# Sharath-girish/Shacira

Hardware: AMD Instinct MI355X
Metric: hash-grid samples/sec fwd+bwd (16 lvl, F=2) (higher is better)
Workload: dtype f32

## Files before the change

### shacira_amd/csrc/api.hip

```cpp
#include <atomic>
#include <cmath>
#include <cstdint>
#include <cstring>

#include "internal.h"

namespace shacira {

struct OptionSlot {
    const char *name;
    int Options::*field;
    int lo, hi;
    std::atomic<int> value;
};
static OptionSlot g_slots[] = {
    {"fwd_variant", &Options::fwd_variant, -1, 9, {-1}},
    {"bwd_variant", &Options::bwd_variant, -1, 1, {-1}},
    {"mlp_variant", &Options::mlp_variant, -1, 1, {-1}},
    {"bwd_compact", &Options::bwd_compact, 0, 1, {1}},
    {"bwd_selective_zero", &Options::bwd_selective_zero, 0, 1, {1}},
    {"bwd_persistent", &Options::bwd_persistent, 0, 1, {1}},
    {"bwd_fork", &Options::bwd_fork, 0, 1, {1}},
    {"bwd_run_pad", &Options::bwd_run_pad, 0, 1, {1}},
    {"bwd_item12", &Options::bwd_item12, -1, 1, {-1}},
    {"bin_acc_kib", &Options::bin_acc_kib, 0, 128, {0}},
    {"bin_batch_mib", &Options::bin_batch_mib, 1, 1 << 20, {1536}},
    {"tiled", &Options::tiled, -1, 1, {-1}},
    {"tiled_lc_fwd", &Options::tiled_lc_fwd, -1, SHACIRA_MAX_LODS, {-1}},
    {"bwd_brick", &Options::bwd_brick, -1, 1, {-1}},
    {"bwd_brick_lo", &Options::bwd_brick_lo, -1, SHACIRA_MAX_LODS, {-1}},
    {"bwd_brick_hi", &Options::bwd_brick_hi, -1, SHACIRA_MAX_LODS, {-1}},
    {"bwd_brick_fork", &Options::bwd_brick_fork, 0, 2, {2}},
    {"bwd_brick_span", &Options::bwd_brick_span, 0, 64, {0}},
    {"fwd_direct", &Options::fwd_direct, -1, 1, {-1}},
    {"bwd_ext_fork", &Options::bwd_ext_fork, 0, 1, {1}},
    {"coord_variant", &Options::coord_variant, -1, 8, {-1}},
    {"triplane_layout", &Options::triplane_layout, -1, 1, {-1}},
};
static thread_local Options tl_options;
const Options &opt() { return tl_options; }
void options_snapshot() {
    for (OptionSlot &sl : g_slots) tl_options.*(sl.field) = sl.value.load(std::memory_order_relaxed);
}
void options_resolve_item12(int value) { tl_options.bwd_item12 = value; }
static bool option_value_ok(const OptionSlot &sl, int v) {
    if (v < sl.lo || v > sl.hi) return false;
    if (!std::strcmp(sl.name, "fwd_variant")) return v == -1 || v == 0 || v == 3 || v == 6 || v == 8 || v == 9;
    if (!std::strcmp(sl.name, "coord_variant")) return v == -1 || v == 0 || v == 3 || v == 8;
    if (!std::strcmp(sl.name, "bin_acc_kib")) return v == 0 || v == 64 || v == 128;
    return true;
}

static int build_level_table(int dim, int num_lods, int feature_dim, int bw, const int32_t *res_host,
                             int64_t table_rows, LevelTable &lt) {
    if (dim != 2 && dim != 3) return SHACIRA_EINVAL;
    if (num_lods < 1 || num_lods > SHACIRA_MAX_LODS) return SHACIRA_EINVAL;
    if (feature_dim < 1) return SHACIRA_EINVAL;
    if (feature_dim % 2 == 1) return SHACIRA_EODD;
    if (bw < 1 || bw > 30) return SHACIRA_EINVAL;
    if (!res_host || table_rows < 0) return SHACIRA_EINVAL;
    std::memset(&lt, 0, sizeof(lt));
    const int32_t cs = (int32_t)std::pow(2.0, (double)bw);
    for (int l = 0; l < num_lods; ++l) {
        const int32_t r = res_host[l];
        if (r < 1) return SHACIRA_EINVAL;
        lt.res[l] = r;
        lt.hi[l] = (float)((double)r - 1.0 - 1e-5);
        lt.dense[l] = level_is_dense(dim, r, cs) ? 1 : 0;
    }
    lt.mask = (uint32_t)cs - 1u;
    lt.num_lods = num_lods;
    lt.feature_dim = feature_dim;
    lt.table_rows = table_rows;
    lt.level_begin = 0;
    lt.level_end = num_lods;
    lt.stage_flags = 0;
    return 0;
}

}

using namespace shacira;

extern "C" {

int shacira_abi_version(void) { return SHACIRA_ABI_VERSION; }

const char *shacira_strerror(int code) {
    switch (code) {
        case 0: return "success";
        case SHACIRA_EINVAL: return "shacira: invalid argument (dim/sizes/bitwidth/null pointer)";
        case SHACIRA_EDTYPE: return "shacira: unsupported scalar type or operator shape";
        case SHACIRA_EODD: return "The codebook feature dimension needs to be a multiple of 2.";
        case SHACIRA_EWORKSPACE: return "shacira: workspace too small";
        default: break;
    }
    if (code > 0) return hipGetErrorString((hipError_t)code);
    return "shacira: unknown error";
}

int shacira_set_option(const char *name, int value) {
    if (!name) return SHACIRA_EINVAL;
    for (OptionSlot &sl : g_slots) {
        if (std::strcmp(name, sl.name)) continue;
        if (!option_value_ok(sl, value)) return SHACIRA_EINVAL;
        sl.value.store(value, std::memory_order_relaxed);
        return 0;
    }
    return SHACIRA_EINVAL;
}

int shacira_get_option(const char *name) {
    if (!name) return SHACIRA_EINVAL;
    for (OptionSlot &sl : g_slots)
        if (!std::strcmp(name, sl.name)) return sl.value.load(std::memory_order_relaxed);
    return SHACIRA_EINVAL;
}

size_t shacira_hashgrid_forward_workspace_bytes(int dim, int64_t num_coords, int num_lods, int feature_dim,
                                                int codebook_bitwidth, const int32_t *resolutions_host,
                                                int64_t table_rows, int dtype) {
    options_snapshot();
    LevelTable lt;
    if (build_level_table(dim, num_lods, feature_dim, codebook_bitwidth, resolutions_host, table_rows, lt)) return 0;
    return hashgrid_forward_workspace(dim, dtype, lt, num_coords);
}

int shacira_hashgrid_forward(int dim, int64_t num_coords, int num_lods, int feature_dim, int codebook_bitwidth,
                             const int32_t *resolutions_host, const int32_t *codebook_first_idx, int64_t table_rows,
                             const float *coords, const void *codebook, int dtype, void *feats, void *workspace,
                             size_t workspace_bytes, void *stream) {
    return shacira_hashgrid_forward_planned(dim, num_coords, num_lods, feature_dim, codebook_bitwidth, resolutions_host,
                                            codebook_first_idx, table_rows, coords, codebook, dtype, feats, nullptr, 0, 0,
                                            workspace, workspace_bytes, stream);
}

size_t shacira_hashgrid_plan_bytes(int dim, int64_t num_coords, int num_lods, int feature_dim, int codebook_bitwidth,
                                   const int32_t *resolutions_host, int64_t table_rows, int dtype) {
    options_snapshot();
    LevelTable lt;
    if (build_level_table(dim, num_lods, feature_dim, codebook_bitwidth, resolutions_host, table_rows, lt)) return 0;
    if (dtype == SHACIRA_F64 || table_rows == 0 || !tiled_supported(dim, dtype, lt, num_coords)) return 0;
    return sample_plan_bytes(dim, num_coords);
}

int shacira_hashgrid_forward_planned(int dim, int64_t num_coords, int num_lods, int feature_dim, int codebook_bitwidth,
                                     const int32_t *resolutions_host, const int32_t *codebook_first_idx, int64_t table_rows,
                                     const float *coords, const void *codebook, int dtype, void *feats, void *plan,
                                     size_t plan_bytes, int plan_flags, void *workspace, size_t workspace_bytes,
                                     void *stream) {
    options_snapshot();
    LevelTable lt;
    int rc = build_level_table(dim, num_lods, feature_dim, codebook_bitwidth, resolutions_host, table_rows, lt);
    if (rc) return rc;
    if (dtype != SHACIRA_F32 && dtype != SHACIRA_F16 && dtype != SHACIRA_F64) return SHACIRA_EDTYPE;
    if (num_coords < 0) return SHACIRA_EINVAL;
    if (num_coords == 0) return 0;
    if (!codebook_first_idx || !coords || !codebook || !feats) return SHACIRA_EINVAL;
    const size_t need = hashgrid_forward_workspace(dim, dtype, lt, num_coords);
    if (need > 0 && (!workspace || workspace_bytes < need)) return SHACIRA_EWORKSPACE;
    const bool sorts = dtype != SHACIRA_F64 && table_rows > 0 && tiled_supported(dim, dtype, lt, num_coords);
    if (plan != nullptr && sorts && plan_bytes < sample_plan_bytes(dim, num_coords)) return SHACIRA_EWORKSPACE;
    if ((plan_flags & ~SHACIRA_PLAN_READY) != 0 || ((plan_flags & SHACIRA_PLAN_READY) != 0 && plan == nullptr)) return SHACIRA_EINVAL;
    return (int)hashgrid_forward_dispatch(dim, dtype, lt, codebook_first_idx, coords, codebook, feats, workspace,
                                          num_coords, (hipStream_t)stream, sorts ? plan : nullptr,
                                          (plan_flags & SHACIRA_PLAN_READY) != 0);
}

int shacira_hashgrid_debug_corners(int dim, int64_t num_coords, int num_lods, int codebook_bitwidth,
                                   const int32_t *resolutions_host, const float *coords, int32_t *corner_rows,
                                   float *corner_weights, void *stream) {
    LevelTable lt;
    int rc = build_level_table(dim, num_lods, 2, codebook_bitwidth, resolutions_host, 0, lt);
    if (rc) return rc;
    if (num_coords < 0 || num_coords * (int64_t)num_lods >= ((int64_t)1 << 31) * 256) return SHACIRA_EINVAL;
    if (num_coords > 0 && (!coords || (!corner_rows && !corner_weights))) return SHACIRA_EINVAL;
    return (int)hashgrid_debug_corners(dim, lt, coords, num_coords, corner_rows, corner_weights, (hipStream_t)stream);
}

size_t shacira_hashgrid_backward_workspace_bytes(int dim, int64_t num_coords, int num_lods, int feature_dim,
                                                 int codebook_bitwidth, const int32_t *resolutions_host,
                                                 int64_t table_rows, int dtype) {
    options_snapshot();
    LevelTable lt;
    if (build_level_table(dim, num_lods, feature_dim, codebook_bitwidth, resolutions_host, table_rows, lt)) return 0;
    return hashgrid_backward_workspace(dim, dtype, lt, num_coords);
}

int shacira_hashgrid_backward(int dim, int64_t num_coords, int num_lods, int feature_dim, int codebook_bitwidth,
                              const int32_t *resolutions_host, const int32_t *codebook_first_idx, int64_t table_rows,
                              const float *coords, const void *grad_output, int dtype, void *grad_codebook,
                              void *workspace, size_t workspace_bytes, void *stream) {
    return shacira_hashgrid_backward_levels(dim, num_coords, num_lods, feature_dim, codebook_bitwidth, resolutions_host,
                                            codebook_first_idx, table_rows, coords, grad_output, dtype, grad_codebook,
                                            0, num_lods, 0, workspace, workspace_bytes, stream);
}

static int backward_call(int dim, int64_t num_coords, int num_lods, int feature_dim, int codebook_bitwidth,
                         const int32_t *resolutions_host, const int32_t *codebook_first_idx, int64_t table_rows,
                         const float *coords, const void *grad_output, int dtype, void *grad_codebook, int level_begin,
                         int level_end, int flags, const void *plan, size_t plan_bytes, void *workspace,
                         size_t workspace_bytes, void *stream);

size_t shacira_hashgrid_backward_planned_workspace_bytes(int dim, int64_t num_coords, int num_lods, int feature_dim,
                                                         int codebook_bitwidth, const int32_t *resolutions_host,
                                                         int64_t table_rows, int dtype) {
    options_snapshot();
    LevelTable lt;
    if (build_level_table(dim, num_lods, feature_dim, codebook_bitwidth, resolutions_host, table_rows, lt)) return 0;
    LevelTable full = lt;
    const bool sorts = dtype != SHACIRA_F64 && table_rows > 0 && tiled_supported(dim, dtype, full, num_coords);
    if (!sorts) return hashgrid_backward_workspace(dim, dtype, lt, num_coords);
    return hashgrid_backward_workspace_planned(dim, dtype, lt, num_coords, true);
}

int shacira_hashgrid_backward_planned(int dim, int64_t num_coords, int num_lods, int feature_dim, int codebook_bitwidth,
                                      const int32_t *resolutions_host, const int32_t *codebook_first_idx, int64_t table_rows,
                                      const float *coords, const void *grad_output, int dtype, void *grad_codebook,
                                      const void *plan, size_t plan_bytes, void *workspace, size_t workspace_bytes,
                                      void *stream) {
    return backward_call(dim, num_coords, num_lods, feature_dim, codebook_bitwidth, resolutions_host, codebook_first_idx,
                         table_rows, coords, grad_output, dtype, grad_codebook, 0, num_lods, 0, plan, plan_bytes, workspace,
                         workspace_bytes, stream);
}

int shacira_hashgrid_backward_levels(int dim, int64_t num_coords, int num_lods, int feature_dim, int codebook_bitwidth,
                                     const int32_t *resolutions_host, const int32_t *codebook_first_idx,
                                     int64_t table_rows, const float *coords, const void *grad_output, int dtype,
                                     void *grad_codebook, int level_begin, int level_end, int flags, void *workspace,
                                     size_t workspace_bytes, void *stream) {
    return backward_call(dim, num_coords, num_lods, feature_dim, codebook_bitwidth, resolutions_host, codebook_first_idx,
                         table_rows, coords, grad_output, dtype, grad_codebook, level_begin, level_end, flags, nullptr, 0,
                         workspace, workspace_bytes, stream);
}

size_t shacira_hashgrid_coords_backward_workspace_bytes(int dim, int64_t num_coords, int num_lods, int feature_dim,
                                                        int codebook_bitwidth, const int32_t *resolutions_host,
                                                        int64_t table_rows, int dtype) {
    (void)dim; (void)num_coords; (void)num_lods; (void)feature_dim; (void)codebook_bitwidth; (void)resolutions_host;
    (void)table_rows; (void)dtype;
    return 0;
}

int shacira_hashgrid_coords_backward(int dim, int64_t num_coords, int num_lods, int feature_dim, int codebook_bitwidth,
                                     const int32_t *resolutions_host, const int32_t *codebook_first_idx, int64_t table_rows,
                                     const float *coords, const void *codebook, const void *grad_output, int dtype,
                                     float *grad_coords, const void *plan, size_t plan_bytes, void *workspace,
                                     size_t workspace_bytes, void *stream) {
    options_snapshot();
    LevelTable lt;
    int rc = build_level_table(dim, num_lods, feature_dim, codebook_bitwidth, resolutions_host, table_rows, lt);
    if (rc) return rc;
    if (dtype != SHACIRA_F32 && dtype != SHACIRA_F16 && dtype != SHACIRA_F64) return SHACIRA_EDTYPE;
    if (num_coords < 0) return SHACIRA_EINVAL;
    if (num_coords == 0) return 0;
    if (!codebook_first_idx || !coords || !codebook || !grad_output || !grad_coords) return SHACIRA_EINVAL;
    const size_t need = shacira_hashgrid_coords_backward_workspace_bytes(dim, num_coords, num_lods, feature_dim,
                                                                         codebook_bitwidth, resolutions_host, table_rows,
                                                                         dtype);
    if (need > 0 && (!workspace || workspace_bytes < need)) return SHACIRA_EWORKSPACE;
    if (plan != nullptr) {
        const bool sorts = dtype != SHACIRA_F64 && table_rows > 0 && tiled_supported(dim, dtype, lt, num_coords);
        if (!sorts) plan = nullptr;
        else if (plan_bytes < sample_plan_bytes(dim, num_coords)) return SHACIRA_EWORKSPACE;
    }
    return (int)hashgrid_coord_grad_dispatch(dim, dtype, lt, codebook_first_idx, coords, codebook, grad_output, grad_coords,
                                             num_coords, (hipStream_t)stream, plan);
}

static int triplane_args(int64_t num_coords, int num_lods, const int32_t *lods_host, int feature_dim, TriplaneArgs &a) {
    if (num_coords < 0 || num_coords > (int64_t)INT32_MAX) return SHACIRA_EINVAL;
    if (num_lods < 1 || num_lods > SHACIRA_TRIPLANE_MAX_LODS || !lods_host) return SHACIRA_EINVAL;
    if (feature_dim < 1 || feature_dim > SHACIRA_TRIPLANE_MAX_FDIM) return SHACIRA_EINVAL;
    std::memset(&a, 0, sizeof(a));
    a.num_lods = num_lods;
    a.fdim = feature_dim;
    for (int l = 0; l < num_lods; ++l) {
        if (lods_host[l] < 0 || lods_host[l] > SHACIRA_TRIPLANE_MAX_LOD) return SHACIRA_EINVAL;
        a.side[l] = (1 << lods_host[l]) + 1;
    }
    return 0;
}

static int triplane_pointers(int num_lods, const float *const *host, TriplaneArgs &a, bool grad) {
    if (!host) return SHACIRA_EINVAL;
    for (int q = 0; q < 3 * num_lods; ++q) {
        if (!host[q]) return SHACIRA_EINVAL;
        if (grad) a.grad[q] = const_cast<float *>(host[q]);
        else a.plane[q] = host[q];
    }
    return 0;
}

size_t shacira_triplane_forward_workspace_bytes(int64_t num_coords, int num_lods, const int32_t *lods_host,
                                                int feature_dim, int multiscale_sum) {
    options_snapshot();
    TriplaneArgs a;
    if (triplane_args(num_coords, num_lods, lods_host, feature_dim, a)) return 0;
    return triplane_forward_workspace(a, num_coords);
}

int shacira_triplane_forward(int64_t num_coords, int num_lods, const int32_t *lods_host, int feature_dim,
                             const float *coords, const float *const *planes_host, int multiscale_sum, float *feats,
                             void *workspace, size_t workspace_bytes, void *stream) {
    options_snapshot();
    TriplaneArgs a;
    if (int rc = triplane_args(num_coords, num_lods, lods_host, feature_dim, a)) return rc;
    if (multiscale_sum != 0 && multiscale_sum != 1) return SHACIRA_EINVAL;
    if (num_coords == 0) return 0;
    if (!coords || !feats) return SHACIRA_EINVAL;
    if (int rc = triplane_pointers(num_lods, planes_host, a, false)) return rc;
    const size_t need = triplane_forward_workspace(a, num_coords);
    if (need > 0 && (!workspace || workspace_bytes < need)) return SHACIRA_EWORKSPACE;
    return (int)triplane_forward_dispatch(a, coords, multiscale_sum, feats, workspace, num_coords, (hipStream_t)stream);
}

size_t shacira_triplane_backward_workspace_bytes(int64_t num_coords, int num_lods, const int32_t *lods_host,
                                                 int feature_dim, int multiscale_sum, int flags) {
    TriplaneArgs a;
    if (triplane_args(num_coords, num_lods, lods_host, feature_dim, a)) return 0;
    if ((flags & SHACIRA_TRIPLANE_GRAD_PLANES) == 0) return 0;
    return triplane_backward_workspace(a, multiscale_sum, num_coords);
}

int shacira_triplane_backward(int64_t num_coords, int num_lods, const int32_t *lods_host, int feature_dim,
                              const float *coords, const float *const *planes_host, const float *grad_output,
                              int multiscale_sum, int flags, float *const *grad_planes_host, float *grad_coords,
                              void *workspace, size_t workspace_bytes, void *stream) {
    TriplaneArgs a;
    if (int rc = triplane_args(num_coords, num_lods, lods_host, feature_dim, a)) return rc;
    if (multiscale_sum != 0 && multiscale_sum != 1) return SHACIRA_EINVAL;
    if (flags <= 0 || (flags & ~(SHACIRA_TRIPLANE_GRAD_PLANES | SHACIRA_TRIPLANE_GRAD_COORDS)) != 0) return SHACIRA_EINVAL;
    const bool planes = (flags & SHACIRA_TRIPLANE_GRAD_PLANES) != 0;
    const bool want_coords = (flags & SHACIRA_TRIPLANE_GRAD_COORDS) != 0;
    if (planes)
        if (int rc = triplane_pointers(num_lods, const_cast<const float *const *>(grad_planes_host), a, true)) return rc;
// ... 539 lines not shown
```

### shacira_amd/csrc/bwd_bin_front.h

```cpp
#pragma once

#include "bwd_bin_types.h"

namespace shacira {

template <typename T, int F, bool GMAX>
__global__ __launch_bounds__(256) void transpose_grad_kernel(const T *__restrict__ go, float *__restrict__ gT,
                                                             int64_t N, int64_t NP, int L, int lb, int le,
                                                             uint32_t *__restrict__ gmax) {
    __shared__ uint32_t s_max[SHACIRA_MAX_LODS];
    if (GMAX && threadIdx.x < SHACIRA_MAX_LODS) s_max[threadIdx.x] = 0;
    struct alignas(sizeof(T) * F) PieceIn { T v[F]; };
    struct alignas(sizeof(float) * F) PieceOut { float v[F]; };
    extern __shared__ __align__(16) unsigned char s_raw_g[];
    PieceOut *s_tile = reinterpret_cast<PieceOut *>(s_raw_g);
    const int pitch = L + 1;
    const int64_t s0 = (int64_t)blockIdx.x * 256;
    const int ns = (int)((N - s0 < 256) ? (N - s0) : 256);
    const PieceIn *in = reinterpret_cast<const PieceIn *>(go) + s0 * L;
    const int total = ns * L;
    for (int e = threadIdx.x; e < total; e += 256) {
        const int sm = e / L, l = e - sm * L;
        const PieceIn p = in[e];
        PieceOut q;
#pragma unroll
        for (int j = 0; j < F; ++j) q.v[j] = Scalar<T>::load(&p.v[j]);
        s_tile[sm * pitch + l] = q;
    }
    __syncthreads();
    PieceOut *out = reinterpret_cast<PieceOut *>(gT);
    for (int l = lb; l < le; ++l) {
        uint32_t m = 0;
        if ((int)threadIdx.x < ns) {
            const PieceOut q = s_tile[threadIdx.x * pitch + l];
            if constexpr (GMAX) {
#pragma unroll
                for (int j = 0; j < F; ++j) {
                    const uint32_t b = __float_as_uint(fabsf(q.v[j]));
                    m = b > m ? b : m;
                }
            }
            float *dst = reinterpret_cast<float *>(out + (int64_t)l * NP + s0 + threadIdx.x);
            if constexpr (F == 2) {
                typedef float f32x2 __attribute__((ext_vector_type(2)));
                f32x2 v = {q.v[0], q.v[1]};
                __builtin_nontemporal_store(v, reinterpret_cast<f32x2 *>(dst));
            } else {
#pragma unroll
                for (int j = 0; j < F; ++j) __builtin_nontemporal_store(q.v[j], dst + j);
            }
        }
        if constexpr (GMAX) {
#pragma unroll
            for (int off = 32; off > 0; off >>= 1) {
                const uint32_t o = __shfl_xor(m, off, 64);
                m = o > m ? o : m;
            }
            if ((threadIdx.x & 63) == 0 && m) atomicMax(&s_max[l], m);
        }
    }
    if constexpr (GMAX) {
        __syncthreads();
        if ((int)threadIdx.x >= lb && (int)threadIdx.x < le && s_max[threadIdx.x])
            atomicMax(&gmax[threadIdx.x], s_max[threadIdx.x]);
    }
}

constexpr int kFrontThreads = 512;
template <int DIM, typename T, int F, bool GMAX, bool COUNT, bool SORTED = false>
__global__ __launch_bounds__(kFrontThreads) void front16_kernel(LevelTable lt, BinPlan plan, const T *__restrict__ go,
                                                                float *__restrict__ gT, const float *__restrict__ coords,
                                                                uint32_t *__restrict__ totals, uint32_t *__restrict__ cnt,
                                                                int64_t N, int64_t NP, int lb, int le, int ts_log2,
                                                                int rounds, uint32_t *__restrict__ gmax, uint32_t cps,
                                                                const float4 *__restrict__ sorted4 = nullptr) {
    constexpr int K = 16 / (int)(sizeof(T) * F);
    constexpr int HE = SHACIRA_MAX_LODS * kMaxLevelBuckets / kFrontThreads;
    constexpr int M = 16 / (4 * F);
    constexpr int M_LOG2 = (M == 2) ? 1 : 0;
    constexpr int UL = 8;
    static_assert(K >= 1 && (M == 1 || M == 2), "16-byte transpose: F = 2 or 4");
    typedef uint32_t u32x4 __attribute__((ext_vector_type(4)));
    typedef float f32x4 __attribute__((ext_vector_type(4)));
    struct alignas(sizeof(float) * F) PieceOut { float v[F]; };
    __shared__ uint32_t s_max[SHACIRA_MAX_LODS];
    __shared__ uint32_t s_idx[SORTED ? kFrontThreads : 1];
    extern __shared__ __align__(16) unsigned char s_raw_g[];
    const int L = lt.num_lods;
    const int TS = 1 << ts_log2;
    const int pitch = TS + 2;
    PieceOut *s_tile = reinterpret_cast<PieceOut *>(s_raw_g);
    uint32_t *s_hist = reinterpret_cast<uint32_t *>(s_raw_g + (size_t)L * pitch * sizeof(PieceOut));
    if (GMAX && threadIdx.x < SHACIRA_MAX_LODS) s_max[threadIdx.x] = 0;
    if constexpr (COUNT)
        for (uint32_t k = threadIdx.x; k < plan.nbl * (uint32_t)kMaxLevelBuckets; k += kFrontThreads) s_hist[k] = 0;
    __syncthreads();
    const int VPR = L / K;
    const int nvec_log2 = ts_log2 - M_LOG2;
    const int q512 = kFrontThreads / VPR, r512 = kFrontThreads % VPR;
    const int sm_first = (int)threadIdx.x / VPR, v_first = (int)threadIdx.x % VPR;
    const int cslots = kFrontThreads >> ts_log2, csm = (int)threadIdx.x & (TS - 1);
    const int cslot = __builtin_amdgcn_readfirstlane((int)threadIdx.x >> ts_log2);
    const int64_t tile0 = (int64_t)blockIdx.x * rounds;
    const int64_t tiles = (N + TS - 1) >> ts_log2;
    uint32_t hsum[HE];
    uint32_t hacc[HE];
    static_assert(!COUNT || kFrontThreads % kMaxLevelBuckets == 0, "a wave maps to one level slot");
    const uint32_t hli0 = (uint32_t)__builtin_amdgcn_readfirstlane((int)(threadIdx.x / kMaxLevelBuckets));
    const uint32_t hb = threadIdx.x % kMaxLevelBuckets;
    auto hcol_of = [&](int j) -> int {
        const uint32_t li = hli0 + (uint32_t)j * (kFrontThreads / kMaxLevelBuckets);
        const uint32_t lc = li < (uint32_t)SHACIRA_MAX_LODS ? li : 0u;
        const uint32_t nbq = li < plan.nbl ? plan.bnb[lc] : 0u, bsq = plan.bstart[lc];
        return (hb < nbq) ? (int)(bsq + hb) : -1;
    };
    if constexpr (COUNT) {
#pragma unroll
        for (int j = 0; j < HE; ++j) {
            hsum[j] = 0;
            hacc[j] = 0;
        }
    }
    float cc[DIM];
    uint32_t cidx = 0;
    auto load_coords = [&](int r) {
        int64_t t = tile0 + r;
        if (t >= tiles) t = tiles - 1;
        const int64_t s0r = t << ts_log2;
        const int nsr = (int)((N - s0r < TS) ? (N - s0r) : TS);
        const int64_t ci = s0r + (csm < nsr ? csm : nsr - 1);
        if constexpr (SORTED) {
            const float4 rc = sorted4[ci];
            cc[0] = rc.x;
            cc[1] = rc.y;
            if constexpr (DIM == 3) cc[2] = rc.z;
            cidx = __float_as_uint(rc.w);
        } else {
#pragma unroll
            for (int a = 0; a < DIM; ++a) cc[a] = coords[ci * DIM + a];
        }
    };
    if constexpr (COUNT || SORTED) {
        if (tile0 < tiles) load_coords(0);
    }
    for (int r = 0; r < rounds && tile0 + r < tiles; ++r) {
        const int64_t s0 = (tile0 + r) << ts_log2;
        const int ns = (int)((N - s0 < TS) ? (N - s0) : TS);
        const int total = ns * VPR;
        const u32x4 *in = reinterpret_cast<const u32x4 *>(go) + (SORTED ? 0 : s0 * VPR);
        if constexpr (SORTED) {
            if (cslot == 0) s_idx[csm] = cidx;
            lds_barrier();
        }
        auto src_of = [&](int e, int smq, int vq) -> const u32x4 * {
            if constexpr (SORTED) return in + (uint32_t)(s_idx[smq] * (uint32_t)VPR + (uint32_t)vq);
            else return in + e;
        };
        u32x4 raw[UL];
        {
            int smq = sm_first, vq = v_first;
#pragma unroll
            for (int u = 0; u < UL; ++u) {
                const int e = (int)threadIdx.x + u * kFrontThreads;
                const bool in_tile = e < total;
                raw[u] = __builtin_nontemporal_load(in_tile ? src_of(e, smq, vq) : src_of(total - 1, ns - 1, VPR - 1));
                smq += q512;
                vq += r512;
                if (vq >= VPR) { vq -= VPR; ++smq; }
            }
        }
        if constexpr (COUNT || SORTED) {
            double t[DIM];
#pragma unroll
            for (int a = 0; a < DIM; ++a) t[a] = axis_unit(cc[a]);
            load_coords(r + 1);
            if (COUNT && csm < ns) {
#pragma unroll 2
                for (uint32_t li = (uint32_t)cslot; li < plan.nbl; li += (uint32_t)cslots)
                    count_level<DIM>(t, plan.cl[li], lt.mask, s_hist + li * kMaxLevelBuckets);
            }
        }
        auto park1 = [&](const u32x4 &rv, int sm, int v) {
            T tv[K * F];
            __builtin_memcpy(tv, &rv, 16);
#pragma unroll
            for (int k = 0; k < K; ++k) {
                PieceOut q;
#pragma unroll
                for (int j = 0; j < F; ++j) q.v[j] = Scalar<T>::load(&tv[k * F + j]);
                s_tile[(v * K + k) * pitch + sm] = q;
            }
        };
        int sm = sm_first, v = v_first;
#pragma unroll
        for (int u = 0; u < UL; ++u) {
            if ((int)threadIdx.x + u * kFrontThreads < total) park1(raw[u], sm, v);
            sm += q512;
            v += r512;
            if (v >= VPR) { v -= VPR; ++sm; }
        }
        for (int e = (int)threadIdx.x + kFrontThreads * UL; e < total; e += kFrontThreads) {
            park1(__builtin_nontemporal_load(src_of(e, sm, v)), sm, v);
            sm += q512;
            v += r512;
            if (v >= VPR) { v -= VPR; ++sm; }
        }
        lds_barrier();
        if constexpr (COUNT) {
            uint32_t *row = cnt + (size_t)(tile0 + r) * plan.total_buckets;
            const bool close = plan.pad > 1u && ((uint32_t)((tile0 + r + 1) % (int64_t)cps) == 0u || tile0 + r + 1 == tiles);
#pragma unroll
            for (int j = 0; j < HE; ++j) {
                const int hc = hcol_of(j);
                if (hc >= 0) {
                    const uint32_t h = s_hist[threadIdx.x + j * kFrontThreads];
                    s_hist[threadIdx.x + j * kFrontThreads] = 0;
                    row[hc] = h;
                    hacc[j] += h;
                    hsum[j] += h;
                    if (close) {
                        hsum[j] += (0u - hacc[j]) & (plan.pad - 1u);
                        hacc[j] = 0;
                    }
                }
            }
        }
        const int work = (le - lb) << nvec_log2;
        for (int idx = threadIdx.x; idx < work; idx += kFrontThreads) {
            const int l = lb + (idx >> nvec_log2), smo = (idx & ((1 << nvec_log2) - 1)) << M_LOG2;
            uint32_t m = 0;
            if (smo < ns) {
                const f32x4 val = *reinterpret_cast<const f32x4 *>(&s_tile[l * pitch + smo]);
                float *dst = gT + ((int64_t)l * NP + s0 + smo) * F;
                if (smo + M <= ns) {
                    if constexpr (sizeof(T) == 4) *reinterpret_cast<f32x4 *>(dst) = val;
                    else __builtin_nontemporal_store(val, reinterpret_cast<f32x4 *>(dst));
                    if constexpr (GMAX) {
#pragma unroll
                        for (int j = 0; j < 4; ++j) {
                            const uint32_t b = __float_as_uint(fabsf(val[j]));
                            m = b > m ? b : m;
                        }
                    }
                } else {
#pragma unroll
                    for (int j = 0; j < F; ++j) {
                        dst[j] = val[j];
                        if constexpr (GMAX) {
                            const uint32_t b = __float_as_uint(fabsf(val[j]));
                            m = b > m ? b : m;
                        }
                    }
                }
            }
            if constexpr (GMAX) {
#pragma unroll
                for (int off = 32; off > 0; off >>= 1) {
                    const uint32_t o = __shfl_xor(m, off, 64);
                    m = o > m ? o : m;
                }
                if ((threadIdx.x & 63) == 0 && m) atomicMax(&s_max[l], m);
            }
        }
        lds_barrier();
    }
    __syncthreads();
    if constexpr (COUNT) {
        uint32_t *mine = totals + (size_t)(blockIdx.x % kTotalShards) * kMaxBuckets;
#pragma unroll
        for (int j = 0; j < HE; ++j) {
            const int hc = hcol_of(j);
            if (hc >= 0 && hsum[j]) atomicAdd(&mine[hc], hsum[j]);
        }
    }
    if constexpr (GMAX) {
        if ((int)threadIdx.x >= lb && (int)threadIdx.x < le && s_max[threadIdx.x])
            atomicMax(&gmax[threadIdx.x], s_max[threadIdx.x]);
    }
}

__global__ __launch_bounds__(1024) void bin_scan_buckets_kernel(const uint32_t *__restrict__ totals,
                                                                uint64_t *__restrict__ base,
                                                                uint32_t *__restrict__ unit_first,
                                                                UnitDesc *__restrict__ unit_desc, uint32_t nb,
                                                                BinPlan plan,
                                                                uint32_t *__restrict__ work_counter,
                                                                unsigned long long *__restrict__ cursor,
                                                                const uint32_t *__restrict__ gmax) {
    __shared__ uint64_t s_items[kMaxBuckets + 2];
    __shared__ uint32_t s_units[kMaxBuckets + 2];
    __shared__ uint64_t s_wave_items[16];
    __shared__ uint32_t s_wave_units[16];
    const uint32_t t = threadIdx.x, lane = t & 63, wave = t >> 6;
    if (t == 0) work_counter[0] = 0;
    uint64_t c[2];
    uint32_t u[2], lv_of[2], ck[2];
#pragma unroll
    for (int k = 0; k < 2; ++k) {
        const uint32_t b = 2 * t + k;
        c[k] = 0u;
        if (b < nb)
            for (int sh = 0; sh < kTotalShards; ++sh) c[k] += totals[(size_t)sh * kMaxBuckets + b];
        uint32_t lvl = plan.blevel[0];
#pragma unroll
        for (uint32_t q = 1; q < SHACIRA_MAX_LODS; ++q)
            if (q < plan.nbl && plan.bstart[q] <= b) lvl = plan.blevel[q];
        lv_of[k] = lvl;
        ck[k] = plan.chunk;
        u[k] = (c[k] >> 32) ? (uint32_t)((c[k] + ck[k] - 1) / ck[k]) : (c[k] ? ((uint32_t)c[k] - 1u) / ck[k] + 1u : 0u);
    }
    uint64_t ci = c[0] + c[1];
    uint32_t ui = u[0] + u[1];
#pragma unroll
    for (int off = 1; off < 64; off <<= 1) {
        const uint64_t nc = __shfl_up(ci, off, 64);
        const uint32_t nu = __shfl_up(ui, off, 64);
        if (lane >= (uint32_t)off) { ci += nc; ui += nu; }
    }
    if (lane == 63) { s_wave_items[wave] = ci; s_wave_units[wave] = ui; }
    __syncthreads();
    uint64_t wc = 0;
    uint32_t wu = 0;
    for (uint32_t w = 0; w < wave; ++w) { wc += s_wave_items[w]; wu += s_wave_units[w]; }
    const uint64_t ex_items = wc + ci - (c[0] + c[1]);
    const uint32_t ex_units = wu + ui - (u[0] + u[1]);
    s_items[2 * t] = ex_items;
    s_items[2 * t + 1] = ex_items + c[0];
    s_units[2 * t] = ex_units;
    s_units[2 * t + 1] = ex_units + u[0];
    if (t == 1023) {
        s_items[kMaxBuckets] = ex_items + c[0] + c[1];
        s_units[kMaxBuckets] = ex_units + u[0] + u[1];
    }
    __syncthreads();
    for (uint32_t b = t; b <= nb; b += 1024) {
        base[b] = s_items[b];
        cursor[b] = s_items[b];
        unit_first[b] = s_units[b];
    }
#pragma unroll
    for (int k = 0; k < 2; ++k) {
        const uint32_t b = 2 * t + k;
        if (b < nb) {
            const uint32_t lvl = lv_of[k];
            const uint32_t gm = (gmax != nullptr && u[k] > 0) ? gmax[lvl] : 0u;
            for (uint32_t q = 0; q < u[k]; ++q) {
                UnitDesc d;
                d.begin = s_items[b] + (uint64_t)q * ck[k];
                const uint64_t bucket_end = s_items[b] + c[k];
                d.end = (d.begin + ck[k] < bucket_end) ? (d.begin + ck[k]) : bucket_end;
                d.bucket = b;
                d.level = lvl;
                d.single = u[k] == 1 ? 1u : 0u;
                d.gmax_bits = gm;
                unit_desc[s_units[b] + q] = d;
            }
        }
    }
}

template <int DIM>
__global__ __launch_bounds__(kBinThreads) void bin_count_levels_kernel(LevelTable lt, BinPlan plan,
                                                                       const float *__restrict__ coords,
                                                                       uint32_t *__restrict__ totals,
                                                                       uint32_t *__restrict__ cnt, int64_t sample0,
                                                                       int64_t N) {
    __shared__ uint32_t s_hist[SHACIRA_MAX_LODS][kMaxLevelBuckets];
    constexpr int kTileD = TileOf<DIM>::value;
    constexpr int SPT = kTileD / kBinThreads;
    const uint32_t tile = blockIdx.x;
    for (uint32_t e = threadIdx.x; e < plan.nbl * kMaxLevelBuckets; e += kBinThreads) (&s_hist[0][0])[e] = 0;
    double t[SPT][DIM];
    bool live[SPT];
#pragma unroll
    for (int u = 0; u < SPT; ++u) {
        const int64_t i = sample0 + (int64_t)tile * kTileD + threadIdx.x + u * kBinThreads;
        live[u] = i < N;
        load_unit_coords<DIM>(coords, i, N, t[u]);
    }
    __syncthreads();
#pragma unroll 1
    for (uint32_t bi = blockIdx.y; bi < plan.nbl; bi += gridDim.y) {
        const uint32_t lvl = plan.blevel[bi];
        const BinLevel bl = plan.lv[lvl];
        const int32_t res = lt.res[lvl];
        const float hi = lt.hi[lvl];
        const bool dense = lt.dense[lvl] != 0;
#pragma unroll
        for (int u = 0; u < SPT; ++u) {
            if (!live[u]) continue;
            if (bl.compact) {
                if constexpr (DIM == 3) {
                    atomicAdd(&s_hist[bi][axis_pos(t[u][2], res, hi) / bl.slab], 2u);
                } else {
                    atomicAdd(&s_hist[bi][compact2d_line(axis_pos(t[u][1], res, hi), (uint32_t)res) / bl.slab], 1u);
                }
                continue;
            }
            uint32_t bk[1 << (DIM - 1)];
            bool ok[1 << (DIM - 1)];
            enumerate_buckets<DIM>(t[u], res, hi, dense, lt.mask, bl, bk, ok);
#pragma unroll
            for (int q = 0; q < (1 << (DIM - 1)); ++q)
                if (ok[q]) atomicAdd(&s_hist[bi][bk[q]], 1u);
        }
    }
    __syncthreads();
    for (uint32_t bi = blockIdx.y; bi < plan.nbl; bi += gridDim.y) {
        const BinLevel bl = plan.lv[plan.blevel[bi]];
        for (uint32_t b = threadIdx.x; b < bl.nb; b += kBinThreads)
        {
            const uint32_t c = (s_hist[bi][b] + plan.pad - 1u) & ~(plan.pad - 1u);
            cnt[(size_t)tile * plan.total_buckets + bl.bucket0 + b] = s_hist[bi][b];
            if (c)
                atomicAdd(&totals[(size_t)((blockIdx.x + blockIdx.y) % kTotalShards) * kMaxBuckets + bl.bucket0 + b], c);
        }
    }
}

__global__ __launch_bounds__(256) void zero_unowned_rows_kernel(float *__restrict__ acc,
                                                                const int32_t *__restrict__ first_idx, LevelTable lt,
                                                                BinPlan plan, uint32_t *__restrict__ words,
                                                                uint32_t nwords) {
    if ((int)blockIdx.y == lt.num_lods) {
        for (uint32_t i = blockIdx.x * 256 + threadIdx.x; i < nwords; i += gridDim.x * 256) words[i] = 0u;
        return;
    }
    const int l = blockIdx.y, F = lt.feature_dim;
    const int64_t level0 = first_idx[l];
    const int64_t start = (l == 0) ? 0 : level0;
    const int64_t end = (l + 1 < lt.num_lods) ? (int64_t)first_idx[l + 1] : lt.table_rows;
    const BinLevel bl = plan.lv[l];
    const bool covered = bl.nb > 0 && bl.dgroup < 0 && lt.dense[l] == 0;
    const int64_t hole_lo = covered ? level0 : end;
    int64_t hole_hi = covered ? level0 + (int64_t)bl.used : end;
    if (hole_hi > end) hole_hi = end;
    const int64_t stride = (int64_t)gridDim.x * 256, t0 = (int64_t)blockIdx.x * 256 + threadIdx.x;
    for (int64_t e = start * F + t0; e < hole_lo * F; e += stride) acc[e] = 0.0f;
    for (int64_t e = hole_hi * F + t0; e < end * F; e += stride) acc[e] = 0.0f;
}

__global__ __launch_bounds__(256) void zero_words_kernel(uint32_t *__restrict__ p, uint32_t n) {
    for (uint32_t i = blockIdx.x * 256 + threadIdx.x; i < n; i += gridDim.x * 256) p[i] = 0u;
}

template <int F> __device__ __forceinline__ void rotate_features(const float (&a)[F], int rot, float (&r)[F]) {
    static_assert(F == 1 || F == 2 || F == 4 || F == 8, "power-of-two feature counts");
#pragma unroll
    for (int k = 0; k < F; ++k) r[k] = a[k];
#pragma unroll
    for (int bit = 1; bit < F; bit <<= 1) {
        int on = rot & bit;
        asm volatile("" : "+v"(on));
        float t[F];
#pragma unroll
        for (int k = 0; k < F; ++k) t[k] = on ? r[(k + bit) & (F - 1)] : r[k];
#pragma unroll
        for (int k = 0; k < F; ++k) r[k] = t[k];
    }
}

}
```

### shacira_amd/csrc/bwd_bin_passes.h

```cpp
#pragma once

#include "bwd_bin_types.h"

namespace shacira {

#ifdef SHACIRA_SCATTER_WAVES
#define SHACIRA_SCATTER_ATTR __attribute__((amdgpu_waves_per_eu(SHACIRA_SCATTER_WAVES)))
#else
#define SHACIRA_SCATTER_ATTR
#endif
template <int DIM, int F, int FMT, bool STREAM = true>
__global__ __launch_bounds__((ScatterThreads<DIM, F, FMT>::value)) SHACIRA_SCATTER_ATTR void bin_scatter_kernel(LevelTable lt, BinPlan plan,
                                                                  const float *__restrict__ coords,
                                                                  const float *__restrict__ gT,
                                                                  unsigned long long *__restrict__ cursor,
                                                                  const uint32_t *__restrict__ cnt, uint32_t cps,
                                                                  uint32_t cnt_rows,
                                                                  typename ItemSel<F, FMT>::type *__restrict__ items,
                                                                  int64_t sample0, int64_t N, int64_t gpitch,
                                                                  float *__restrict__ zero_acc,
                                                                  const int32_t *__restrict__ first_idx,
                                                                  const uint32_t *__restrict__ unit_first,
                                                                  int cstride = DIM) {
    typedef typename ItemSel<F, FMT>::type ItemT;
    constexpr bool H = FMT == 1;
    constexpr bool P12 = FMT == 2;
    static_assert(!P12 || (DIM == 3 && F == 2), "12-byte units: 3-D, F = 2");
    constexpr int NP = 1 << (DIM - 1);
    constexpr int kTileD = TileOf<DIM>::value;
    constexpr int kThreads = ScatterThreads<DIM, F, FMT>::value;
    constexpr int SPT = kTileD / kThreads;
    constexpr int kScatterSplit = ScatterSplit<ItemT>::value;
    constexpr int kStage = kTileD * NP / kScatterSplit;
    static_assert(kStage % 2 == 0, "two-slot items never straddle a window");
    extern __shared__ __align__(16) unsigned char s_raw[];
    ItemT *s_items = reinterpret_cast<ItemT *>(s_raw);
    uint8_t *s_bucket = reinterpret_cast<uint8_t *>(s_items + (kScatterSplit == 1 ? plan.stage_cap : (uint32_t)kStage));
    __shared__ uint32_t s_hist[kMaxLevelBuckets];
    __shared__ uint32_t s_start[kMaxLevelBuckets + 1];
    __shared__ uint64_t s_gbase[kMaxLevelBuckets];

#ifdef SCATTER_LEVEL_FAST
    const uint32_t tile = blockIdx.y, bi = blockIdx.x;
#else
    const uint32_t tile = blockIdx.x, bi = blockIdx.y;
#endif
    const uint32_t lvl = plan.blevel[bi];
    const BinLevel bl = plan.lv[lvl];
    if (threadIdx.x < kMaxLevelBuckets) s_hist[threadIdx.x] = 0;
    __syncthreads();
    const int32_t res = lt.res[lvl];
    const float hi = lt.hi[lvl];
    const bool dense = lt.dense[lvl] != 0;

    PairSlot ps[SPT][NP];
    uint32_t rank[SPT][NP];
    float fx[SPT];
    float g[SPT][F];
    float fyz[SPT][2];
    const bool compact = bl.compact != 0;
    constexpr uint32_t kCompactSlots = (DIM == 3) ? 2u : 1u;
    float craw[SPT][DIM], graw[SPT][F];
#pragma unroll
    for (int u = 0; u < SPT; ++u) {
        int64_t i = sample0 + (int64_t)tile * kTileD + threadIdx.x + u * kThreads;
        i = i < N ? i : N - 1;
#ifdef ABL_NO_LOAD
        i = (i * 2654435761ll) & 1023;
#endif
#pragma unroll
        for (int a = 0; a < DIM; ++a) craw[u][a] = coords[i * cstride + a];
        const float *gp = gT + ((int64_t)lvl * gpitch + i) * F;
        if constexpr (F == 2) {
            const float2 v = *reinterpret_cast<const float2 *>(gp);
            graw[u][0] = v.x; graw[u][1] = v.y;
        } else {
#pragma unroll
            for (int j = 0; j < F; ++j) graw[u][j] = gp[j];
        }
    }
    const bool reserver = threadIdx.x >= 64 && threadIdx.x - 64 < bl.nb;
    unsigned long long run_base = 0ull;
    if (reserver) {
        const uint32_t gb = bl.bucket0 + threadIdx.x - 64;
        const uint32_t *row = cnt + (size_t)tile * cps * plan.total_buckets + gb;
        uint32_t c = 0;
        for (uint32_t k = 0; k < cps && tile * cps + k < cnt_rows; ++k) c += row[(size_t)k * plan.total_buckets];
        c = (c + plan.pad - 1u) & ~(plan.pad - 1u);
#ifdef ABL_NO_CURSOR
        if (c) run_base = cursor[gb] + (unsigned long long)tile * c;
#else
        if (c) run_base = atomicAdd(&cursor[gb], (unsigned long long)c);
#endif
    }
#pragma unroll
    for (int u = 0; u < SPT; ++u) {
        const int k = threadIdx.x + u * kThreads;
        const int64_t i = sample0 + (int64_t)tile * kTileD + k;
        const bool live = i < N;
        double t[DIM];
#pragma unroll
        for (int a = 0; a < DIM; ++a) t[a] = axis_unit(craw[u][a]);
#pragma unroll
        for (int j = 0; j < F; ++j) g[u][j] = graw[u][j];
        if (compact) {
            if constexpr (DIM == 3) {
                int32_t pp[3];
                float ff[3], gg[3];
#pragma unroll
                for (int a = 0; a < 3; ++a) axis_transform(t[a], res, hi, pp[a], ff[a], gg[a]);
                const uint32_t r = (uint32_t)res, b = (uint32_t)pp[2] / bl.slab;
                const uint32_t local = ((uint32_t)pp[2] - b * bl.slab) * r * r + (uint32_t)pp[1] * r + (uint32_t)pp[0];
                fx[u] = ff[0];
                fyz[u][0] = ff[1];
                fyz[u][1] = ff[2];
#pragma unroll
                for (int q = 0; q < NP; ++q) {
                    ps[u][q].bucket = b;
                    ps[u][q].key = 0;
                    ps[u][q].wrest = 0.0f;
                }
                ps[u][0].key = local | (1u << 26);
            } else {
                int32_t pp[2];
                float ff[2], gg[2];
#pragma unroll
                for (int a = 0; a < 2; ++a) axis_transform(t[a], res, hi, pp[a], ff[a], gg[a]);
                const uint32_t r = (uint32_t)res, b = compact2d_line((uint32_t)pp[1], r) / bl.slab;
                const uint32_t local = ((uint32_t)pp[1] - b * bl.slab) * r + (uint32_t)pp[0];
                fx[u] = ff[0];
                fyz[u][0] = ff[1];
                fyz[u][1] = 0.0f;
                ps[u][0].bucket = b;
                ps[u][0].key = local | (1u << 26);
                ps[u][0].wrest = 0.0f;
                ps[u][1].bucket = b;
                ps[u][1].key = 0;
                ps[u][1].wrest = 0.0f;
            }
        } else {
            enumerate_pairs<DIM>(t, res, hi, dense, lt.mask, bl, plan.BR, fx[u], ps[u]);
        }
#pragma unroll
        for (int q = 0; q < NP; ++q) {
            if (!live) ps[u][q].key = 0;
            rank[u][q] = (ps[u][q].key >> 26) ? atomicAdd(&s_hist[ps[u][q].bucket], compact ? kCompactSlots : 1u) : 0u;
        }
    }
    lds_barrier();
    if (threadIdx.x < 64) {
        const uint32_t lane = threadIdx.x;
        const uint32_t pm = plan.pad - 1u;
        const uint32_t c0 = (2 * lane < bl.nb) ? ((s_hist[2 * lane] + pm) & ~pm) : 0u;
        const uint32_t c1 = (2 * lane + 1 < bl.nb) ? ((s_hist[2 * lane + 1] + pm) & ~pm) : 0u;
        uint32_t incl = c0 + c1;
#pragma unroll
        for (int off = 1; off < 64; off <<= 1) {
            const uint32_t nbr = __shfl_up(incl, off, 64);
            if (lane >= (uint32_t)off) incl += nbr;
        }
        const uint32_t excl = incl - (c0 + c1);
        if (2 * lane < bl.nb) s_start[2 * lane] = excl;
        if (2 * lane + 1 < bl.nb) s_start[2 * lane + 1] = excl + c0;
        if (lane == 63) s_start[bl.nb] = incl;
    }
    lds_barrier();
    if (kScatterSplit == 1 && plan.pad > 1u && threadIdx.x < bl.nb) {
        const uint32_t b = threadIdx.x;
        for (uint32_t pos = s_start[b] + s_hist[b]; pos < s_start[b + 1]; ++pos) {
            uint32_t *w = reinterpret_cast<uint32_t *>(&s_items[pos]);
#pragma unroll
            for (int k = 0; k < (int)(sizeof(ItemT) / 4); ++k) w[k] = 0u;
            s_bucket[pos] = (uint8_t)b;
        }
    }
    const uint32_t staged = s_start[bl.nb];
    const uint32_t n_win = (kScatterSplit == 1) ? 1u : (staged + (uint32_t)kStage - 1u) / (uint32_t)kStage;
    for (uint32_t wi = 0; wi < n_win; ++wi) {
    const uint32_t w0 = wi * (uint32_t)kStage;
#pragma unroll
    for (int u = 0; u < SPT; ++u) {
#pragma unroll
        for (int q = 0; q < NP; ++q) {
            if (ps[u][q].key >> 26) {
                const uint32_t gp = s_start[ps[u][q].bucket] + rank[u][q];
                if (kScatterSplit > 1 && gp - w0 >= (uint32_t)kStage) continue;
                const uint32_t pos = gp - w0;
                if constexpr (H && F == 4) {
                    ItemH4 it;
                    it.key = ps[u][q].key;
                    it.fx = fx[u];
                    if (compact) {
                        it.p2 = __float_as_uint(fyz[u][0]);
                        it.p3 = __float_as_uint(fyz[u][1]);
                        s_items[pos] = it;
                        ItemH4 it2;
                        it2.key = 0;
                        it2.fx = 0.0f;
                        it2.p2 = float2_to_half2_bits(g[u][0], g[u][1]);
                        it2.p3 = float2_to_half2_bits(g[u][2], g[u][3]);
                        s_items[pos + 1] = it2;
                        s_bucket[pos] = (uint8_t)ps[u][q].bucket;
                        s_bucket[pos + 1] = (uint8_t)ps[u][q].bucket;
                    } else {
                        const float w = ps[u][q].wrest;
                        it.p2 = float2_to_half2_bits(g[u][0] * w, g[u][1] * w);
                        it.p3 = float2_to_half2_bits(g[u][2] * w, g[u][3] * w);
                        s_items[pos] = it;
                        s_bucket[pos] = (uint8_t)ps[u][q].bucket;
                    }
                    continue;
                }
                if constexpr (P12) {
                    if (compact) {
                        Item12 u0, u1;
                        u0.w[0] = ps[u][q].key;
                        u0.w[1] = __float_as_uint(fx[u]);
                        u0.w[2] = __float_as_uint(fyz[u][0]);
                        u1.w[0] = __float_as_uint(fyz[u][1]);
                        u1.w[1] = __float_as_uint(g[u][0]);
                        u1.w[2] = __float_as_uint(g[u][1]);
                        s_items[pos] = u0;
                        s_items[pos + 1] = u1;
                        s_bucket[pos] = (uint8_t)ps[u][q].bucket;
                        s_bucket[pos + 1] = (uint8_t)ps[u][q].bucket;
                    } else {
                        s_items[pos] = pack_item12(ps[u][q].key, fx[u], dense, g[u][0] * ps[u][q].wrest, g[u][1] * ps[u][q].wrest);
                        s_bucket[pos] = (uint8_t)ps[u][q].bucket;
                    }
                    continue;
                }
                if constexpr (H && F == 2) {
                    if (compact) {
                        ItemHC c;
                        c.key = ps[u][q].key;
                        c.fx = (uint16_t)(fx[u] * 65536.0f);
                        c.fy = (uint16_t)(fyz[u][0] * 65536.0f);
                        c.fz = (uint16_t)(fyz[u][1] * 65536.0f);
                        c.pad = 0;
                        c.g = __floats2half2_rn(g[u][0], g[u][1]);
                        *reinterpret_cast<ItemHC *>(&s_items[pos]) = c;
                        s_bucket[pos] = (uint8_t)ps[u][q].bucket;
                        s_bucket[pos + 1] = (uint8_t)ps[u][q].bucket;
                    } else {
                        ItemH it;
                        it.key = pack_half_key(ps[u][q].key, fx[u], dense);
                        it.a = __floats2half2_rn(g[u][0] * ps[u][q].wrest, g[u][1] * ps[u][q].wrest);
                        s_items[pos] = it;
                        s_bucket[pos] = (uint8_t)ps[u][q].bucket;
                    }
                    continue;
                }
                if constexpr (!H && !P12) {
                Item<F> it;
                it.key = ps[u][q].key;
                it.fx = fx[u];
                if constexpr (DIM == 2 && !H) {
                    if (compact) {
                        uint32_t w0, w1;
                        pack_compact2d(ps[u][q].key, fx[u], fyz[u][0], w0, w1);
                        it.key = w0;
                        it.fx = __uint_as_float(w1);
#pragma unroll
                        for (int j = 0; j < F; ++j) it.a[j] = g[u][j];
                        *reinterpret_cast<Item<F> *>(&s_items[pos]) = it;
                        s_bucket[pos] = (uint8_t)ps[u][q].bucket;
                        continue;
                    }
                }
                if (compact) {
                    if constexpr (F == 2) {
                        it.a[0] = fyz[u][0];
                        it.a[1] = fyz[u][1];
                        *reinterpret_cast<Item<F> *>(&s_items[pos]) = it;
                        Item<F> it2;
                        it2.key = 0;
                        it2.fx = g[u][0];
                        it2.a[0] = g[u][1];
                        it2.a[1] = 0.0f;
                        *reinterpret_cast<Item<F> *>(&s_items[pos + 1]) = it2;
                        s_bucket[pos] = (uint8_t)ps[u][q].bucket;
                        s_bucket[pos + 1] = (uint8_t)ps[u][q].bucket;
                    } else if constexpr (F == 4) {
                        it.a[0] = fyz[u][0];
                        it.a[1] = fyz[u][1];
                        it.a[2] = g[u][0];
                        it.a[3] = g[u][1];
                        *reinterpret_cast<Item<F> *>(&s_items[pos]) = it;
                        Item<F> it2;
                        it2.key = 0;
                        it2.fx = g[u][2];
                        it2.a[0] = g[u][3];
                        it2.a[1] = 0.0f; it2.a[2] = 0.0f; it2.a[3] = 0.0f;
                        *reinterpret_cast<Item<F> *>(&s_items[pos + 1]) = it2;
                        s_bucket[pos] = (uint8_t)ps[u][q].bucket;
                        s_bucket[pos + 1] = (uint8_t)ps[u][q].bucket;
                    }
                } else {
#pragma unroll
                    for (int j = 0; j < F; ++j) it.a[j] = g[u][j] * ps[u][q].wrest;
                    *reinterpret_cast<Item<F> *>(&s_items[pos]) = it;
                    s_bucket[pos] = (uint8_t)ps[u][q].bucket;
                }
                }
            }
        }
    }
    if (wi == 0) {
        if (reserver) s_gbase[threadIdx.x - 64] = run_base;
        __syncthreads();
    } else {
        lds_barrier();
    }
    const uint32_t in_window = (kScatterSplit == 1 || staged - w0 < (uint32_t)kStage) ? (staged - w0) : (uint32_t)kStage;
#ifndef ABL_NO_STORE
    for (uint32_t pos = threadIdx.x; pos < in_window; pos += kThreads) {
        const uint32_t b = s_bucket[pos];
        store_item_nt<STREAM>(items + s_gbase[b] + (w0 + pos - s_start[b]), s_items[pos]);
    }
#endif
    if (kScatterSplit > 1 && wi + 1u < n_win) lds_barrier();
    }
    if (zero_acc != nullptr && !dense) {
        for (uint32_t b = tile; b < bl.nb; b += plan.num_tiles) {
            const uint32_t gb = bl.bucket0 + b;
            if (unit_first[gb + 1] - unit_first[gb] == 1u) continue;
            const uint32_t row0 = b * bl.rows_pb;
            const uint32_t nrows = (bl.used - row0 < bl.rows_pb) ? (bl.used - row0) : bl.rows_pb;
            float *dst = zero_acc + ((int64_t)first_idx[lvl] + row0) * F;
            for (uint32_t e = threadIdx.x; e < nrows * (uint32_t)F; e += kThreads) dst[e] = 0.0f;
        }
    }
}

#ifdef CONSUME_TRACE
__device__ unsigned long long g_consume_trace[16384 * 8];
__device__ unsigned int g_consume_trace_n;
#define CTRACE(k) do { if (threadIdx.x == 0) ctr[k] = wall_clock64(); } while (0)
#else
#define CTRACE(k) do { } while (0)
#endif
template <int F, bool FX, int FMT, class Hook>
__device__ __forceinline__ void consume_unit(const LevelTable &lt, const BinPlan &plan, const int32_t *__restrict__ first_idx,
                                             const UnitDesc d, const typename ItemSel<F, FMT>::type *__restrict__ items,
                                             float *__restrict__ grad_table, int force_atomic, int headroom, double *s_acc,
                                             Hook &&hook, __half *__restrict__ half_out = nullptr) {
    constexpr bool H = FMT == 1;
    constexpr bool P12 = FMT == 2;
    const uint32_t gb = (uint32_t)__builtin_amdgcn_readfirstlane((int)d.bucket);
    const uint32_t lvl = (uint32_t)__builtin_amdgcn_readfirstlane((int)d.level);
    const BinLevel bl = plan.lv[lvl];
    const uint32_t b = gb - bl.bucket0;
    const uint32_t r1 = (uint32_t)lt.res[lvl];
    const bool two_d = plan.pairs == 2u;
    const uint32_t row0 = bl.compact ? b * bl.slab * (two_d ? r1 : r1 * r1) : b * bl.rows_pb;
    const uint32_t nrows = (bl.used - row0 < bl.rows_pb) ? (bl.used - row0) : bl.rows_pb;

    FxScale fx{1.0, 1.0, false};
    if constexpr (FX) fx = fx_scale_of(d.gmax_bits, headroom);
    unsigned long long *s_fix = reinterpret_cast<unsigned long long *>(s_acc);
#ifdef CONSUME_TRACE
    unsigned long long ctr[8] = {0, 0, 0, 0, 0, 0, 0, 0};
    struct TraceOut {
        unsigned long long *c; UnitDesc dd;
        __device__ ~TraceOut() {
            if (threadIdx.x == 0) {
                c[5] = wall_clock64();
                const unsigned int slot = atomicAdd(&g_consume_trace_n, 1u);
                if (slot < 16384u) {
                    unsigned long long *o = g_consume_trace + (size_t)slot * 8;
                    o[0] = ((unsigned long long)dd.level << 32) | dd.bucket;
                    o[1] = dd.end - dd.begin;
                    for (int k = 0; k < 6; ++k) o[2 + k] = c[k];
                }
            }
        }
    } trace_out{ctr, d};
#endif
    CTRACE(0);
    auto zero_image = [&]() {
        for (uint32_t e = threadIdx.x; e < nrows * F; e += kConsumeThreads) s_acc[e] = 0.0;
        lds_barrier();
    };
    const uint64_t begin = d.begin, end = d.end;
    auto stream = [&](uint64_t first, uint64_t lim, uint64_t stride, auto &&load, auto &&proc) {
        uint64_t p0 = first;
        load(p0);
        CTRACE(1);
        zero_image();
        CTRACE(2);
        proc();
        CTRACE(3);
        hook();
        for (p0 += stride; p0 < lim; p0 += stride) {
            load(p0);
            proc();
        }
        CTRACE(4);
    };
    const int rot = (int)(threadIdx.x & (F - 1));
    auto add_row = [&](uint32_t row, const float (&vr)[F], float w) {
#pragma unroll
        for (int jj = 0; jj < F; ++jj) {
            const int j = (jj + rot) & (F - 1);
            const float c = vr[jj] * w;
            if (FX && fx.fixed) atomicAdd(&s_fix[row * F + j], fx_encode(c, fx.scale));
            else atomicAdd(&s_acc[row * F + j], (double)c);
        }
    };
#ifdef ABL_CONSUME_STREAM_ONLY
    uint32_t abl_sink = 0;
#endif
    auto add_pair = [&](uint32_t ra, uint32_t rb, bool va, bool vb, float fxv, const float (&a)[F]) {
#ifdef ABL_CONSUME_STREAM_ONLY
        abl_sink ^= ra ^ rb ^ (uint32_t)va ^ (uint32_t)vb ^ __float_as_uint(fxv) ^ __float_as_uint(a[0]) ^ __float_as_uint(a[F - 1]);
        if (abl_sink == 0x12345678u) s_fix[ra] = abl_sink;
        return;
#endif
        float ar[F];
        rotate_features<F>(a, rot, ar);
        if (va) add_row(ra, ar, 1.0f - fxv);
        if (vb) add_row(rb, ar, fxv);
    };
    const uint32_t r2 = r1 * r1;
    auto add_compact = [&](uint32_t base_row, float fxx, float fyy, float fzz, const float (&gg)[F]) {
        const float gxx = 1.0f - fxx, gyy = 1.0f - fyy, gzz = 1.0f - fzz;
        const float wxy[4] = {gxx * gyy, gxx * fyy, fxx * gyy, fxx * fyy};
        float gr[F];
        rotate_features<F>(gg, rot, gr);
#pragma unroll
        for (int c = 0; c < 8; ++c) {
            const uint32_t row = base_row + ((c >> 2) & 1) + ((c >> 1) & 1) * r1 + (c & 1) * r2;
            if (row >= nrows) continue;
            add_row(row, gr, wxy[c >> 1] * ((c & 1) ? fzz : gzz));
        }
    };
    typedef uint32_t u32x4 __attribute__((ext_vector_type(4)));
    typedef uint32_t u32x2 __attribute__((ext_vector_type(2)));
    if constexpr ((F == 2 || F == 4) && !H && !P12) {
        if (bl.compact && two_d) {
            const Item<F> *itf = reinterpret_cast<const Item<F> *>(items);
            constexpr int UD = 8;
            Item<F> it[UD];
            stream(begin + threadIdx.x, end, (uint64_t)kConsumeThreads * UD,
                   [&](uint64_t p0) {
#pragma unroll
                       for (int u = 0; u < UD; ++u) {
                           const uint64_t pp = p0 + (uint64_t)u * kConsumeThreads;
                           if (pp < end) it[u] = load_item_nt<F, FX>(itf + pp);
                           else it[u].key = 0;
                       }
                   },
                   [&]() {
#pragma unroll
                       for (int u = 0; u < UD; ++u) {
                           if (!(it[u].key & (1u << 13))) continue;
                           uint32_t local, qx, qy;
                           unpack_compact2d(it[u].key, __float_as_uint(it[u].fx), local, qx, qy);
                           const float q = 1.0f / 33554432.0f;
                           const float fxx = (float)qx * q, fyy = (float)qy * q;
                           const float gxx = 1.0f - fxx, gyy = 1.0f - fyy;
                           float ar[F];
                           rotate_features<F>(it[u].a, rot, ar);
                           if (local + r1 + 1u < nrows) {
                               add_row(local, ar, gxx * gyy);
                               if (qx) add_row(local + 1u, ar, fxx * gyy);
                               if (qy) {
                                   add_row(local + r1, ar, gxx * fyy);
                                   if (qx) add_row(local + r1 + 1u, ar, fxx * fyy);
                               }
                           } else {
                               if (local < nrows) add_row(local, ar, gxx * gyy);
                               if (qx && local + 1u < nrows) add_row(local + 1u, ar, fxx * gyy);
                               if (qy && local + r1 < nrows) add_row(local + r1, ar, gxx * fyy);
                           }
                       }
                   });
            lds_barrier();
            const int64_t grow0d = (int64_t)first_idx[lvl] + row0;
            for (uint32_t e = threadIdx.x; e < nrows * F; e += kConsumeThreads) {
                const int64_t grow = grow0d + e / F;
                if ((uint64_t)grow >= (uint64_t)lt.table_rows) continue;
                const float v = (FX && fx.fixed) ? fx_decode(s_fix[e], fx.inv) : (float)s_acc[e];
                if (v != 0.0f) unsafeAtomicAdd(grad_table + grow * F + (e % F), v);
            }
            return;
        }
    }
    if constexpr (F == 2 || F == 4) {
        if (bl.compact) {
            constexpr int UC = 2;
            const uint64_t first = begin + 2ull * threadIdx.x, stride = 2ull * kConsumeThreads * UC;
            if constexpr (P12) {
                Item12 ia[UC], ib[UC];
                uint64_t pcur = 0;
                stream(first, end, stride,
                       [&](uint64_t p0) {
                           pcur = p0;
#pragma unroll
                           for (int u = 0; u < UC; ++u) {
                               const uint64_t p = p0 + 2ull * u * kConsumeThreads;
                               const uint64_t pc = (p + 1 < end) ? p : begin;
                               ia[u] = load_item12_nt(items + pc);
                               ib[u] = load_item12_nt(items + pc + 1);
                           }
                       },
                       [&]() {
#pragma unroll
                           for (int u = 0; u < UC; ++u) {
                               if (pcur + 2ull * u * kConsumeThreads + 1 >= end) continue;
                               if (!(ia[u].w[0] & (1u << 26))) continue;
                               const float gg[F] = {__uint_as_float(ib[u].w[1]), __uint_as_float(ib[u].w[2])};
                               add_compact(ia[u].w[0] & 0x1FFFu, __uint_as_float(ia[u].w[1]), __uint_as_float(ia[u].w[2]),
                                           __uint_as_float(ib[u].w[0]), gg);
                           }
                       });
            } else if constexpr (H && F == 4) {
                u32x4 va[UC], vb2[UC];
                stream(first, end, stride,
                       [&](uint64_t p0) {
#pragma unroll
                           for (int u = 0; u < UC; ++u) {
                               const uint64_t p = p0 + 2ull * u * kConsumeThreads;
                               va[u] = u32x4{0u, 0u, 0u, 0u};
                               vb2[u] = va[u];
                               if (p + 1 < end) {
                                   va[u] = __builtin_nontemporal_load(reinterpret_cast<const u32x4 *>(items + p));
                                   vb2[u] = __builtin_nontemporal_load(reinterpret_cast<const u32x4 *>(items + p + 1));
                               }
                           }
                       },
                       [&]() {
#pragma unroll
                           for (int u = 0; u < UC; ++u) {
                               if (!(va[u][0] & (1u << 26))) continue;
                               const float2 g01 = half2_bits_to_float2(vb2[u][2]);
                               const float2 g23 = half2_bits_to_float2(vb2[u][3]);
                               const float gg[F] = {g01.x, g01.y, g23.x, g23.y};
                               add_compact(va[u][0] & 0x1FFFu, __uint_as_float(va[u][1]), __uint_as_float(va[u][2]),
                                           __uint_as_float(va[u][3]), gg);
                           }
                       });
            } else if constexpr (H) {
                ItemHC rec[UC];
                stream(first, end, stride,
                       [&](uint64_t p0) {
#pragma unroll
                           for (int u = 0; u < UC; ++u) {
                               const uint64_t p = p0 + 2ull * u * kConsumeThreads;
                               rec[u].key = 0;
                               if (p + 1 < end) {
                                   const u32x4 v = __builtin_nontemporal_load(reinterpret_cast<const u32x4 *>(items + p));
                                   __builtin_memcpy(&rec[u], &v, 16);
                               }
                           }
                       },
                       [&]() {
#pragma unroll
                           for (int u = 0; u < UC; ++u) {
                               if (!(rec[u].key & (1u << 26))) continue;
                               const float2 gf = __half22float2(rec[u].g);
                               const float gg[F] = {gf.x, gf.y};
                               const float q = 1.0f / 65536.0f;
                               add_compact(rec[u].key & 0x1FFFu, ((float)rec[u].fx + 0.5f) * q, ((float)rec[u].fy + 0.5f) * q,
                                           ((float)rec[u].fz + 0.5f) * q, gg);
                           }
                       });
            } else {
                const Item<F> *itf = reinterpret_cast<const Item<F> *>(items);
                Item<F> ia[UC], ib[UC];
                stream(first, end, stride,
                       [&](uint64_t p0) {
#pragma unroll
                           for (int u = 0; u < UC; ++u) {
                               const uint64_t p = p0 + 2ull * u * kConsumeThreads;
                               if constexpr (sizeof(Item<F>) == 16) {
                                   if (p + 1 < end) {
                                       ia[u] = load_item_nt<F, FX>(itf + p);
                                       ib[u] = load_item_nt<F, FX>(itf + p + 1);
                                   } else {
                                       ia[u].key = 0;
                                   }
                               } else {
                                   const uint64_t pc = (p + 1 < end) ? p : begin;
                                   ia[u] = load_item_nt<F, FX>(itf + pc);
                                   ib[u] = load_item_nt<F, FX>(itf + pc + 1);
                               }
                           }
                           if constexpr (sizeof(Item<F>) != 16) {
#pragma unroll
                               for (int u = 0; u < UC; ++u)
                                   if (p0 + 2ull * u * kConsumeThreads + 1 >= end) ia[u].key = 0;
                           }
                       },
                       [&]() {
#pragma unroll
                           for (int u = 0; u < UC; ++u) {
                               if (!(ia[u].key & (1u << 26))) continue;
                               float gg[F];
                               if constexpr (F == 2) {
                                   gg[0] = ib[u].fx; gg[1] = ib[u].a[0];
                               } else {
                                   gg[0] = ia[u].a[2]; gg[1] = ia[u].a[3]; gg[2] = ib[u].fx; gg[3] = ib[u].a[0];
                               }
                               add_compact(ia[u].key & 0x1FFFu, ia[u].fx, ia[u].a[0], ia[u].a[1], gg);
                           }
                       });
            }
            lds_barrier();
            const int64_t grow0c = (int64_t)first_idx[lvl] + row0;
            for (uint32_t e = threadIdx.x; e < nrows * F; e += kConsumeThreads) {
                const int64_t grow = grow0c + e / F;
                if ((uint64_t)grow >= (uint64_t)lt.table_rows) continue;
                const float v = (FX && fx.fixed) ? fx_decode(s_fix[e], fx.inv) : (float)s_acc[e];
                if (v != 0.0f) unsafeAtomicAdd(grad_table + grow * F + (e % F), v);
            }
            return;
        }
    }
    constexpr int UN = 8;
    if constexpr (P12) {
        Item12 it[UN];
        uint64_t pcur = 0;
        stream(begin + threadIdx.x, end, (uint64_t)kConsumeThreads * UN,
               [&](uint64_t p0) {
                   pcur = p0;
#pragma unroll
                   for (int u = 0; u < UN; ++u) {
                       const uint64_t pp = p0 + (uint64_t)u * kConsumeThreads;
// ... 426 lines not shown
```

### shacira_amd/csrc/bwd_bin_types.h

```cpp
#pragma once

#include "internal.h"

namespace shacira {

#ifndef SHACIRA_KTILE
#define SHACIRA_KTILE 1024
#endif
#ifndef SHACIRA_KBIN
#define SHACIRA_KBIN 512
#endif
constexpr int kTile = SHACIRA_KTILE;
#ifndef SHACIRA_TILE2D_MUL
#define SHACIRA_TILE2D_MUL 2
#endif
template <int DIM> struct TileOf { static constexpr int value = (DIM == 2) ? SHACIRA_TILE2D_MUL * kTile : kTile; };
static inline int tile_samples(int dim) { return dim == 2 ? SHACIRA_TILE2D_MUL * kTile : kTile; }
constexpr int kBinThreads = SHACIRA_KBIN;
#ifndef SHACIRA_KSCATTER3D
#define SHACIRA_KSCATTER3D 1024
#endif
template <int DIM, int F, int FMT> struct ScatterThreads {
    static constexpr int value = (DIM == 3 && F == 2 && FMT != 1) ? SHACIRA_KSCATTER3D : kBinThreads;
};
constexpr int kConsumeThreads = 1024;
constexpr int kMaxBuckets = 2048;
constexpr int kMaxLevelBuckets = 128;
constexpr int kTotalShards = 16;

struct BinLevel {
    uint32_t nb;
    uint32_t bucket0;
    uint32_t rows_pb;
    uint32_t G;
    uint64_t magicG;
    uint32_t used;
    uint32_t shift;
    int32_t dgroup;
    uint32_t drow0;
    uint32_t compact;
    uint32_t slab;
    uint32_t chunk;
};

struct CountLevel {
    int32_t res;
    float hi;
    uint32_t kind;
    uint32_t shift;
    uint32_t m_lo, m_hi;
};

struct BinPlan {
    BinLevel lv[SHACIRA_MAX_LODS];
    CountLevel cl[SHACIRA_MAX_LODS];
    uint32_t total_buckets;
    uint32_t BR;
    uint32_t num_tiles;
    uint32_t pairs;
    uint32_t chunk;
    uint32_t chunk_min;
    uint32_t nbl;
    uint32_t pad;
    uint32_t stage_cap;
    uint32_t blevel[SHACIRA_MAX_LODS];
    uint32_t bstart[SHACIRA_MAX_LODS];
    uint32_t bnb[SHACIRA_MAX_LODS];
    uint32_t ngroups;
    uint32_t gmask[SHACIRA_MAX_LODS];
    uint32_t grows[SHACIRA_MAX_LODS];
};

template <int F> struct alignas(F == 2 ? 16 : 8) Item {
    uint32_t key;
    float fx;
    float a[F];
};

struct alignas(8) ItemH {
    uint32_t key;
    __half2 a;
};
struct alignas(16) ItemHC {
    uint32_t key;
    uint16_t fx, fy, fz, pad;
    __half2 g;
};
struct alignas(16) ItemH4 {
    uint32_t key;
    float fx;
    uint32_t p2, p3;
};
struct alignas(4) Item12 {
    uint32_t w[3];
};
template <int F, int FMT> struct ItemSel { typedef Item<F> type; };
template <> struct ItemSel<2, 1> { typedef ItemH type; };
template <> struct ItemSel<4, 1> { typedef ItemH4 type; };
template <> struct ItemSel<2, 2> { typedef Item12 type; };

__device__ __forceinline__ Item12 pack_item12(uint32_t key, float fx, bool dense, float a0, float a1) {
    const uint32_t ra = key & 0x1FFFu, rb = (key >> 13) & 0x1FFFu;
    const uint32_t vb = (key >> 27) & 1u;
    const uint32_t code = dense ? (vb ? 14u : 15u) : (32u - (uint32_t)__clz((int)(ra ^ rb)));
    uint32_t q = (uint32_t)(fx * 2097152.0f + 0.5f);
    q = q > 2097151u ? 2097151u : q;
    Item12 it;
    it.w[0] = ra | (code << 13) | ((q >> 6) << 17);
    it.w[1] = ((__float_as_uint(a0) + 4u) & ~7u) | ((q >> 3) & 7u);
    it.w[2] = ((__float_as_uint(a1) + 4u) & ~7u) | (q & 7u);
    return it;
}
__device__ __forceinline__ void unpack_item12(const uint32_t (&w)[3], uint32_t &ra, uint32_t &rb, bool &va, bool &vb, float &fx,
                                              float (&a)[2]) {
    const uint32_t code = (w[0] >> 13) & 15u;
    ra = w[0] & 0x1FFFu;
    rb = code >= 14u ? ((ra + 1u) & 0x1FFFu) : (ra ^ ((1u << code) - 1u));
    va = code != 0u;
    vb = code != 0u && code != 15u;
    const uint32_t q = ((w[0] >> 17) << 6) | ((w[1] & 7u) << 3) | (w[2] & 7u);
    fx = (float)q * (1.0f / 2097152.0f);
    a[0] = __uint_as_float(w[1] & ~7u);
    a[1] = __uint_as_float(w[2] & ~7u);
}
template <bool STREAM = true> __device__ __forceinline__ void store_item_nt(Item12 *p, const Item12 &it) {
    __builtin_nontemporal_store(it.w[0], &p->w[0]);
    __builtin_nontemporal_store(it.w[1], &p->w[1]);
    __builtin_nontemporal_store(it.w[2], &p->w[2]);
}
__device__ __forceinline__ Item12 load_item12_nt(const Item12 *p) {
    Item12 it;
    it.w[0] = __builtin_nontemporal_load(&p->w[0]);
    it.w[1] = __builtin_nontemporal_load(&p->w[1]);
    it.w[2] = __builtin_nontemporal_load(&p->w[2]);
    return it;
}

#ifdef SHACIRA_SCATTER_SPLIT
template <class ItemT> struct ScatterSplit { static constexpr int value = SHACIRA_SCATTER_SPLIT; };
#else
template <class ItemT> struct ScatterSplit { static constexpr int value = 1; };
template <> struct ScatterSplit<Item<4>> { static constexpr int value = 4; };
#endif

__device__ __forceinline__ uint32_t pack_half_key(uint32_t key, float fx, bool dense) {
    const uint32_t ra = key & 0x1FFFu, rb = (key >> 13) & 0x1FFFu;
    const uint32_t kx = dense ? 0u : (32u - (uint32_t)__clz((int)(ra ^ rb)));
    const uint32_t fq = (uint32_t)(fx * 8192.0f);
    return ra | (kx << 13) | (((key >> 26) & 3u) << 17) | ((fq > 8191u ? 8191u : fq) << 19);
}
__device__ __forceinline__ void unpack_half_key(uint32_t k, uint32_t &ra, uint32_t &rb, bool &va, bool &vb, float &fx) {
    ra = k & 0x1FFFu;
    const uint32_t kx = (k >> 13) & 15u;
    rb = kx ? (ra ^ ((1u << kx) - 1u)) : ((ra + 1u) & 0x1FFFu);
    va = (k >> 17) & 1u;
    vb = (k >> 18) & 1u;
    fx = ((float)(k >> 19) + 0.5f) * (1.0f / 8192.0f);
}
__device__ __forceinline__ uint32_t float2_to_half2_bits(float a, float b) {
    return (uint32_t)__half_as_ushort(__float2half_rn(a)) | ((uint32_t)__half_as_ushort(__float2half_rn(b)) << 16);
}
__device__ __forceinline__ float2 half2_bits_to_float2(uint32_t bits) {
    return make_float2(__half2float(__ushort_as_half((unsigned short)(bits & 0xFFFFu))),
                       __half2float(__ushort_as_half((unsigned short)(bits >> 16))));
}
template <bool STREAM = true> __device__ __forceinline__ void store_item_nt(ItemH4 *p, const ItemH4 &it) {
    typedef uint32_t u32x4 __attribute__((ext_vector_type(4)));
    u32x4 v;
    __builtin_memcpy(&v, &it, 16);
    *reinterpret_cast<u32x4 *>(p) = v;
}
template <bool STREAM = true> __device__ __forceinline__ void store_item_nt(ItemH *p, const ItemH &it) {
    typedef uint32_t u32x2 __attribute__((ext_vector_type(2)));
    u32x2 v;
    __builtin_memcpy(&v, &it, 8);
#ifdef SHACIRA_HALF_NT
    __builtin_nontemporal_store(v, reinterpret_cast<u32x2 *>(p));
#else
    *reinterpret_cast<u32x2 *>(p) = v;
#endif
}

struct alignas(16) UnitDesc {
    uint64_t begin, end;
    uint32_t bucket;
    uint32_t level;
    uint32_t single;
    uint32_t gmax_bits;
};

__device__ __forceinline__ void lds_barrier() { asm volatile("s_waitcnt lgkmcnt(0)\n\ts_barrier" ::: "memory"); }

template <bool STREAM = true, int F> __device__ __forceinline__ void store_item_nt(Item<F> *p, const Item<F> &it) {
    typedef uint32_t u32x4 __attribute__((ext_vector_type(4)));
    if constexpr (sizeof(Item<F>) == 16) {
        u32x4 v;
        __builtin_memcpy(&v, &it, 16);
        if constexpr (STREAM) __builtin_nontemporal_store(v, reinterpret_cast<u32x4 *>(p));
        else *reinterpret_cast<u32x4 *>(p) = v;
    } else {
        typedef uint32_t u32x2 __attribute__((ext_vector_type(2)));
        static_assert(sizeof(Item<F>) % 8 == 0, "item size");
        u32x2 *q = reinterpret_cast<u32x2 *>(p);
        u32x2 d[sizeof(Item<F>) / 8];
        __builtin_memcpy(d, &it, sizeof(Item<F>));
#pragma unroll
        for (int k = 0; k < (int)(sizeof(Item<F>) / 8); ++k) __builtin_nontemporal_store(d[k], q + k);
    }
}

template <int F, bool STREAM = true> __device__ __forceinline__ Item<F> load_item_nt(const Item<F> *p) {
    Item<F> it;
    typedef uint32_t u32x4 __attribute__((ext_vector_type(4)));
    if constexpr (sizeof(Item<F>) == 16) {
        u32x4 v;
        if constexpr (STREAM) v = __builtin_nontemporal_load(reinterpret_cast<const u32x4 *>(p));
        else v = *reinterpret_cast<const u32x4 *>(p);
        __builtin_memcpy(&it, &v, 16);
    } else {
        typedef uint32_t u32x2 __attribute__((ext_vector_type(2)));
        const u32x2 *q = reinterpret_cast<const u32x2 *>(p);
        u32x2 d[sizeof(Item<F>) / 8];
#pragma unroll
        for (int k = 0; k < (int)(sizeof(Item<F>) / 8); ++k) d[k] = q[k];
        __builtin_memcpy(&it, d, sizeof(Item<F>));
    }
    return it;
}

struct PairSlot {
    uint32_t bucket;
    uint32_t key;
    float wrest;
};

template <int DIM>
__device__ __forceinline__ void enumerate_pairs(const double (&t)[DIM], int32_t res, float hi, bool dense,
                                                uint32_t mask, const BinLevel &bl, uint32_t BR, float &fx,
                                                PairSlot (&out)[1 << (DIM - 1)]) {
    int32_t p[DIM];
    float f[DIM], g[DIM];
#pragma unroll
    for (int a = 0; a < DIM; ++a) axis_transform(t[a], res, hi, p[a], f[a], g[a]);
    fx = f[0];
    const uint32_t ux = (uint32_t)p[0];
    const uint32_t r = (uint32_t)res;
    constexpr int NP = 1 << (DIM - 1);
    uint32_t hyv[2] = {0u, 0u}, hzv[2] = {0u, 0u};
    if (!dense) {
        hyv[0] = (uint32_t)p[1] * kPrimeY;
        hyv[1] = hyv[0] + kPrimeY;
        if constexpr (DIM == 3) {
            hzv[0] = (uint32_t)p[2] * kPrimeZ;
            hzv[1] = hzv[0] + kPrimeZ;
        }
    }
#pragma unroll
    for (int q = 0; q < NP; ++q) {
        const int dy = (DIM == 3) ? ((q >> 1) & 1) : (q & 1);
        const int dz = (DIM == 3) ? (q & 1) : 0;
        float w = dy ? f[1] : g[1];
        if constexpr (DIM == 3) w = w * (dz ? f[2] : g[2]);
        out[q].wrest = w;
        const uint32_t uy = (uint32_t)p[1] + dy;
        uint32_t uz = 0;
        if constexpr (DIM == 3) uz = (uint32_t)p[2] + dz;
        if (dense) {
            bool ok = uy < r;
            uint32_t line = uy;
            if constexpr (DIM == 3) {
                ok = ok && uz < r;
                line += uz * r;
            }
            const uint32_t b = (uint32_t)(((uint64_t)line * bl.magicG) >> 40);
            const uint32_t ra = (line - b * bl.G) * r + ux;
            const uint32_t va = ok ? 1u : 0u;
            const uint32_t vb = (ok && (ux + 1u) < r) ? 1u : 0u;
            out[q].bucket = ok ? b : 0u;
            out[q].key = (ra & 0x1FFFu) | (((ra + 1u) & 0x1FFFu) << 13) | (va << 26) | (vb << 27);
        } else {
            uint32_t h = hyv[dy];
            if constexpr (DIM == 3) h ^= hzv[dz];
            const uint32_t rowA = (ux ^ h) & mask;
            const uint32_t rowB = ((ux + 1u) ^ h) & mask;
            out[q].bucket = rowA >> bl.shift;
            out[q].key = (rowA & (BR - 1u)) | ((rowB & (BR - 1u)) << 13) | (3u << 26);
        }
    }
}

template <int DIM>
__device__ __forceinline__ void enumerate_buckets(const double (&t)[DIM], int32_t res, float hi, bool dense, uint32_t mask,
                                                  const BinLevel &bl, uint32_t (&bucket)[1 << (DIM - 1)],
                                                  bool (&valid)[1 << (DIM - 1)]) {
    int32_t p[DIM];
    float f, g;
#pragma unroll
    for (int a = 1; a < DIM; ++a) axis_transform(t[a], res, hi, p[a], f, g);
    const uint32_t r = (uint32_t)res;
    constexpr int NP = 1 << (DIM - 1);
#pragma unroll
    for (int q = 0; q < NP; ++q) {
        const int dy = (DIM == 3) ? ((q >> 1) & 1) : (q & 1);
        const int dz = (DIM == 3) ? (q & 1) : 0;
        const uint32_t uy = (uint32_t)p[1] + dy;
        uint32_t uz = 0;
        if constexpr (DIM == 3) uz = (uint32_t)p[2] + dz;
        if (dense) {
            bool ok = uy < r;
            uint32_t line = uy;
            if constexpr (DIM == 3) {
                ok = ok && uz < r;
                line += uz * r;
            }
            valid[q] = ok;
            bucket[q] = ok ? (uint32_t)(((uint64_t)line * bl.magicG) >> 40) : 0u;
        } else {
            uint32_t h = uy * kPrimeY;
            if constexpr (DIM == 3) h ^= uz * kPrimeZ;
            valid[q] = true;
            bucket[q] = (h & mask) >> bl.shift;
        }
    }
}

__device__ __forceinline__ uint32_t compact2d_line(uint32_t py, uint32_t res) { return py < res - 2u ? py : res - 2u; }

__device__ __forceinline__ void pack_compact2d(uint32_t local, float fx, float fy, uint32_t &w0, uint32_t &w1) {
    uint32_t qx = __float2uint_rn(fx * 33554432.0f), qy = __float2uint_rn(fy * 33554432.0f);
    qx = qx > 33554431u ? 33554431u : qx;
    qy = qy > 33554431u ? 33554431u : qy;
    w0 = (local & 0x1FFFu) | (1u << 13) | ((qx >> 7) << 14);
    w1 = ((qx & 127u) << 25) | qy;
}
__device__ __forceinline__ void unpack_compact2d(uint32_t w0, uint32_t w1, uint32_t &local, uint32_t &qx, uint32_t &qy) {
    local = w0 & 0x1FFFu;
    qx = ((w0 >> 14) << 7) | (w1 >> 25);
    qy = w1 & 0x1FFFFFFu;
}

__device__ __forceinline__ uint32_t axis_pos(double t, int32_t res, float hi) {
    float x = (float)((double)res * t);
    x = fmaxf(0.0f, fminf(hi, x));
    return (uint32_t)(int32_t)floorf(x);
}

template <int DIM>
__device__ __forceinline__ void count_level(const double (&t)[DIM], const CountLevel cl, uint32_t mask, uint32_t *hist) {
    if (cl.kind == 1u) {
        if constexpr (DIM == 3) {
            const uint32_t pz = axis_pos(t[2], cl.res, cl.hi);
            const uint32_t b = cl.m_lo ? (__umul24(pz, cl.m_lo) >> 18) : pz / cl.m_hi;
            atomicAdd(hist + b, 2u);
        } else {
            const uint32_t py = compact2d_line(axis_pos(t[1], cl.res, cl.hi), (uint32_t)cl.res);
            const uint32_t b = cl.m_lo ? (__umul24(py, cl.m_lo) >> 18) : py / cl.m_hi;
            atomicAdd(hist + b, 1u);
        }
    } else if (cl.kind == 0u) {
        const uint32_t hy0 = axis_pos(t[1], cl.res, cl.hi) * kPrimeY, hy1 = hy0 + kPrimeY;
        if constexpr (DIM == 3) {
            const uint32_t hz0 = axis_pos(t[2], cl.res, cl.hi) * kPrimeZ, hz1 = hz0 + kPrimeZ;
            atomicAdd(hist + (((hy0 ^ hz0) & mask) >> cl.shift), 1u);
            atomicAdd(hist + (((hy0 ^ hz1) & mask) >> cl.shift), 1u);
            atomicAdd(hist + (((hy1 ^ hz0) & mask) >> cl.shift), 1u);
            atomicAdd(hist + (((hy1 ^ hz1) & mask) >> cl.shift), 1u);
        } else {
            atomicAdd(hist + ((hy0 & mask) >> cl.shift), 1u);
            atomicAdd(hist + ((hy1 & mask) >> cl.shift), 1u);
        }
// ... 50 lines not shown
```

### shacira_amd/csrc/hashgrid_bwd_bin.hip

```cpp
#include <mutex>

#include <cstring>

#include "bwd_bin_types.h"
#include "bwd_bin_front.h"
#include "bwd_bin_passes.h"
#include "bwd_brick.h"
#include <hip/hip_ext.h>

namespace shacira {

static inline size_t align_up(size_t v, size_t a) { return (v + a - 1) / a * a; }

static void make_plan(int dim, int dtype, const LevelTable &lt, int64_t n_batch, BinPlan &plan, int acc_kib,
                      bool one_image_compact, uint32_t skip_mask = 0u, int64_t n_call = 0);
static inline bool half_items(int dtype, const LevelTable &lt);
static inline int item_format(int dim, int dtype, const LevelTable &lt, int64_t n);
static inline size_t item_unit_bytes(int fmt, const LevelTable &lt);
#ifndef SHACIRA_RUN_ALIGN
#define SHACIRA_RUN_ALIGN 64
#endif
#ifndef SHACIRA_PAD_HALF
#define SHACIRA_PAD_HALF 0
#endif
#ifndef SHACIRA_FX_MIN
#define SHACIRA_FX_MIN (1 << 17)
#endif
#ifndef SHACIRA_PERSIST_MIN
#define SHACIRA_PERSIST_MIN (1 << 16)
#endif
static inline bool one_image_compact_rule(int64_t n_total) { return n_total >= ((int64_t)1 << 17); }

static bool bin_feasible(int dim, int dtype, const LevelTable &lt, int acc_kib) {
    const int F = lt.feature_dim;
    if (F != 2 && F != 4) return false;
    const uint32_t BR = (uint32_t)acc_kib * 128u / (uint32_t)F;
    for (int l = 0; l < lt.num_lods; ++l) {
        const uint32_t res = (uint32_t)lt.res[l];
        if (lt.dense[l]) {
            if (res > BR) return false;
        } else {
            uint32_t bits = 0;
            while ((1u << bits) <= res) ++bits;
            if ((1u << bits) > BR && (lt.mask + 1u) > BR) return false;
        }
    }
    BinPlan plan;
    make_plan(dim, dtype, lt, kTile, plan, acc_kib, false);
    if (plan.total_buckets + (uint32_t)lt.num_lods > (uint32_t)kMaxBuckets) return false;
    for (int l = 0; l < lt.num_lods; ++l)
        if (plan.lv[l].nb > (uint32_t)kMaxLevelBuckets) return false;
    return true;
}

static int choose_acc_kib(int dim, int dtype, const LevelTable &lt, int64_t n) {
    const int kib = opt().bin_acc_kib;
    if (kib != 0) return kib;
    const int64_t pairs = (int64_t)1 << (dim - 1);
    const bool large = dim == 3 ? n >= ((int64_t)1 << 17) : n * pairs > ((int64_t)1 << 21);
    if (large || !bin_feasible(dim, dtype, lt, 64)) return 128;
    BinPlan big;
    make_plan(dim, dtype, lt, kTile, big, 128, false);
    return big.nbl == 0 ? 128 : 64;
}

bool bin_supported(int dim, const LevelTable &lt);

bool bin_all_direct(int dim, const LevelTable &lt) {
    if (!bin_supported(dim, lt)) return false;
    BinPlan plan;
    make_plan(dim, SHACIRA_F32, lt, kTile, plan, 128, false);
    return plan.nbl == 0 && plan.ngroups > 0;
}

bool bin_supported(int dim, const LevelTable &lt) {
    const int kib = opt().bin_acc_kib;
    return bin_feasible(dim, SHACIRA_F32, lt, kib ? kib : 128);
}

static void make_plan_uncached(int dim, int dtype, const LevelTable &lt, int64_t n_batch, BinPlan &plan, int acc_kib,
                               bool one_image_compact, uint32_t skip_mask, int64_t n_call);

static void make_plan(int dim, int dtype, const LevelTable &lt, int64_t n_batch, BinPlan &plan, int acc_kib,
                      bool one_image_compact, uint32_t skip_mask, int64_t n_call) {
    if (n_call <= 0) n_call = n_batch;
    struct Key {
        int dim, dtype, acc_kib, oic, compact, run_pad, item12, fmt;
        uint32_t skip_mask;
        int64_t n_batch;
        LevelTable lt;
    };
    struct Entry {
        bool valid = false;
        Key key;
        BinPlan plan;
    };
    constexpr int kEntries = 8;
    thread_local Entry cache[kEntries];
    thread_local int next = 0;
    Key k;
    std::memset(&k, 0, sizeof(k));
    k.dim = dim; k.dtype = dtype; k.acc_kib = acc_kib; k.oic = one_image_compact ? 1 : 0; k.compact = opt().bwd_compact;
    k.run_pad = opt().bwd_run_pad;
    k.item12 = opt().bwd_item12;
    k.skip_mask = skip_mask;
    k.fmt = item_format(dim, dtype, lt, n_call);
    k.n_batch = n_batch;
    std::memcpy(&k.lt, &lt, sizeof(LevelTable));
    for (int e = 0; e < kEntries; ++e) {
        if (cache[e].valid && std::memcmp(&cache[e].key, &k, sizeof(Key)) == 0) {
            plan = cache[e].plan;
            return;
        }
    }
    make_plan_uncached(dim, dtype, lt, n_batch, plan, acc_kib, one_image_compact, skip_mask, n_call);
    Entry &slot = cache[next];
    next = (next + 1) % kEntries;
    slot.key = k;
    slot.plan = plan;
    slot.valid = true;
}

static void make_plan_uncached(int dim, int dtype, const LevelTable &lt, int64_t n_batch, BinPlan &plan, int acc_kib,
                               bool one_image_compact, uint32_t skip_mask, int64_t n_call) {
    if (one_image_compact) {
        make_plan_uncached(dim, dtype, lt, n_batch, plan, acc_kib, false, skip_mask, n_call);
        if (plan.nbl == 0) return;
    }
    const int F = lt.feature_dim;
    const uint32_t BR = (uint32_t)acc_kib * 128u / (uint32_t)F;
    uint32_t shift = 0;
    while ((1u << shift) < BR) ++shift;
    uint32_t nbk = 0;
    plan.nbl = 0;
    plan.ngroups = 0;
    for (int l = 0; l < lt.num_lods; ++l) {
        BinLevel &bl = plan.lv[l];
        const uint64_t res = (uint64_t)lt.res[l];
        bl.bucket0 = nbk;
        bl.shift = shift;
        bl.dgroup = -1;
        bl.drow0 = 0;
        bl.compact = 0;
        bl.slab = 0;
        if (l < lt.level_begin || l >= lt.level_end || ((skip_mask >> l) & 1u)) {
            bl.nb = 0;
            bl.used = 0;
            bl.rows_pb = 0;
            bl.G = 1;
            bl.magicG = 0;
            bl.bucket0 = 0xFFFFFFFFu;
            continue;
        }
        if (lt.dense[l]) {
            const uint64_t lines = (dim == 3) ? res * res : res;
            bl.used = (uint32_t)(lines * res);
            bl.G = (uint32_t)(BR / res);
            if (bl.G > lines) bl.G = (uint32_t)lines;
            bl.rows_pb = (uint32_t)(bl.G * res);
            bl.nb = (uint32_t)((lines + bl.G - 1) / bl.G);
            bl.magicG = (((uint64_t)1 << 40) + bl.G - 1) / bl.G;
            const bool cm = (F == 2 || F == 4) && opt().bwd_compact != 0 && (dim == 3 || !half_items(dtype, lt));
            const uint64_t plane_rows = (dim == 3) ? res * res : res;
            const uint64_t planes = cm ? BR / plane_rows : 0;
            if (planes >= 2 && res >= 3 && (bl.used > BR || (one_image_compact && dim == 3))) {
                const uint32_t slab = (uint32_t)planes - 1;
                const uint32_t nbz = ((uint32_t)res - 2u) / slab + 1u;
                if (nbz <= (uint32_t)kMaxLevelBuckets) {
                    bl.compact = 1;
                    bl.slab = slab;
                    bl.rows_pb = (slab + 1u) * (uint32_t)plane_rows;
                    bl.nb = nbz;
                }
            }
        } else {
            bl.used = lt.mask + 1u;
            bl.rows_pb = (bl.used < BR) ? bl.used : BR;
            bl.nb = (bl.used + BR - 1) / BR;
            bl.G = 1;
            bl.magicG = 0;
        }
        if (bl.nb == 1 && bl.used <= BR && !bl.compact) {
            uint32_t gi = 0;
            while (gi < plan.ngroups && plan.grows[gi] + bl.used > BR) ++gi;
            if (gi == plan.ngroups) {
                plan.gmask[gi] = 0;
                plan.grows[gi] = 0;
                ++plan.ngroups;
            }
            bl.dgroup = (int32_t)gi;
            bl.drow0 = plan.grows[gi];
            plan.grows[gi] += bl.used;
            plan.gmask[gi] |= 1u << l;
            bl.bucket0 = 0xFFFFFFFFu;
            bl.nb = 0;
        } else {
            plan.blevel[plan.nbl++] = (uint32_t)l;
            nbk += bl.nb;
        }
    }
    if (plan.ngroups > 1) {
        int dl[SHACIRA_MAX_LODS], ndl = 0;
        for (int l = 0; l < lt.num_lods; ++l)
            if (plan.lv[l].dgroup >= 0) dl[ndl++] = l;
        uint32_t nmask[SHACIRA_MAX_LODS] = {0}, nrows[SHACIRA_MAX_LODS] = {0}, row0[SHACIRA_MAX_LODS] = {0};
        int grp_of[SHACIRA_MAX_LODS];
        uint32_t g = 0;
        int in_group = 0, k = 0;
        bool ok = true;
        for (; k < ndl; ++k) {
            const uint32_t used = plan.lv[dl[k]].used;
            const int left_levels = ndl - k, left_groups = (int)plan.ngroups - (int)g;
            const int quota = (left_levels + in_group + left_groups - 1) / left_groups;
            if (in_group > 0 && (nrows[g] + used > BR || in_group >= quota)) {
                ++g;
                in_group = 0;
                if (g >= plan.ngroups) { ok = false; break; }
            }
            if (nrows[g] + used > BR) { ok = false; break; }
            grp_of[k] = (int)g;
            row0[k] = nrows[g];
            nrows[g] += used;
            nmask[g] |= 1u << dl[k];
            ++in_group;
        }
        if (ok) {
            for (uint32_t q = 0; q < plan.ngroups; ++q) {
                plan.gmask[q] = nmask[q];
                plan.grows[q] = nrows[q];
            }
            for (int q = 0; q < ndl; ++q) {
                plan.lv[dl[q]].dgroup = grp_of[q];
                plan.lv[dl[q]].drow0 = row0[q];
            }
        }
    }
    for (uint32_t q = 0; q < (uint32_t)SHACIRA_MAX_LODS; ++q) {
        plan.bstart[q] = q < plan.nbl ? plan.lv[plan.blevel[q]].bucket0 : 0u;
        plan.bnb[q] = q < plan.nbl ? plan.lv[plan.blevel[q]].nb : 0u;
    }
    plan.total_buckets = nbk;
    plan.BR = BR;
    plan.num_tiles = (uint32_t)((n_batch + tile_samples(dim) - 1) / tile_samples(dim));
    plan.pairs = 1u << (dim - 1);
    uint64_t chunk = (uint64_t)n_batch * plan.pairs / 48 + 1024;
    if (chunk < 8192) chunk = 8192;
    if (chunk > (1u << 22)) chunk = 1u << 22;
    plan.pad = 1;
    {
        const int fmt_p = item_format(dim, dtype, lt, n_call);
        const size_t unit = item_unit_bytes(fmt_p, lt);
        const uint32_t tile_units = (uint32_t)tile_samples(dim) * plan.pairs;
        uint32_t maxnb = 0;
        for (uint32_t q = 0; q < plan.nbl; ++q) maxnb = plan.lv[plan.blevel[q]].nb > maxnb ? plan.lv[plan.blevel[q]].nb : maxnb;
        bool windows = false;
#ifdef SHACIRA_SCATTER_SPLIT
        windows = SHACIRA_SCATTER_SPLIT > 1;
#endif
        if (opt().bwd_run_pad != 0 && !windows && plan.nbl > 0 && n_call >= SHACIRA_FX_MIN &&
            ((fmt_p != 1 && (unit == 16 || unit == 12)) || (SHACIRA_PAD_HALF && fmt_p == 1 && (unit == 8 || unit == 16)))) {
            const uint32_t P = unit == 12 ? (uint32_t)(SHACIRA_RUN_ALIGN / 4) : (uint32_t)(SHACIRA_RUN_ALIGN / unit);
            const size_t staged = (size_t)(tile_units + maxnb * (P - 1u)) * (unit + 1);
            if (staged <= (size_t)78 * 1024 || (size_t)tile_units * (unit + 1) > (size_t)78 * 1024) plan.pad = P;
        }
        plan.stage_cap = tile_units + maxnb * (plan.pad - 1u);
    }
    const uint32_t cmask = plan.pad > 2u ? plan.pad - 1u : 1u;
    plan.chunk = (uint32_t)chunk & ~cmask;
    for (uint32_t q = 0; q < plan.nbl; ++q) {
        BinLevel &bl = plan.lv[plan.blevel[q]];
        bl.chunk = plan.chunk;
        CountLevel &c = plan.cl[q];
        c.res = lt.res[plan.blevel[q]];
        c.hi = lt.hi[plan.blevel[q]];
        c.shift = bl.shift;
        c.m_lo = (uint32_t)bl.magicG;
        c.m_hi = (uint32_t)(bl.magicG >> 32);
        c.kind = lt.dense[plan.blevel[q]] ? 2u : 0u;
        if (bl.compact) {
            const uint32_t m = ((1u << 18) + bl.slab - 1u) / bl.slab;
            bool exact = m < (1u << 18) || bl.slab == 1;
            for (uint32_t pz = 0; pz < (uint32_t)c.res && exact; ++pz) exact = ((pz * m) >> 18) == pz / bl.slab;
            c.kind = 1u;
            c.m_lo = exact ? m : 0u;
            c.m_hi = bl.slab;
        }
    }
    plan.chunk_min = plan.chunk;
}

static inline bool half_items(int dtype, const LevelTable &lt) {
    return dtype == SHACIRA_F16 && (lt.feature_dim == 2 || lt.feature_dim == 4);
}
static inline int item_format(int dim, int dtype, const LevelTable &lt, int64_t n) {
    if (half_items(dtype, lt)) return 1;
    if (dim == 3 && lt.feature_dim == 2 && dtype == SHACIRA_F32 && n >= SHACIRA_FX_MIN && opt().bwd_item12 == 1) return 2;
    return 0;
}
static inline size_t item_unit_bytes(int fmt, const LevelTable &lt) {
    if (fmt == 1) return lt.feature_dim == 2 ? 8 : 16;
    if (fmt == 2) return 12;
    return 8 + 4 * (size_t)lt.feature_dim;
}

static int64_t bin_batch_samples(int dim, int dtype, const LevelTable &lt, int64_t n) {
    const size_t item = item_unit_bytes(item_format(dim, dtype, lt, n), lt);
    BinPlan plan;
    make_plan(dim, dtype, lt, kTile, plan, choose_acc_kib(dim, dtype, lt, n), one_image_compact_rule(n));
    const size_t per_sample = (size_t)(plan.nbl ? plan.nbl : 1) * (1u << (dim - 1)) * item;
    int64_t cap = (int64_t)(((size_t)opt().bin_batch_mib << 20) / per_sample);
    cap = cap / tile_samples(dim) * tile_samples(dim);
    if (cap < tile_samples(dim)) cap = tile_samples(dim);
    return n < cap ? n : cap;
}

struct BinWorkspace {
    float *gT;
    unsigned char *items;
    uint32_t *totals;
    uint32_t *gmax;
    uint64_t *base;
    unsigned long long *cursor;
    uint32_t *cnt;
    uint32_t *unit_first;
    UnitDesc *unit_desc;
    uint32_t *work_counter;
    float *acc32;
    size_t bytes;
};

static inline int64_t level_pitch(int64_t n) { return (n + 1) & ~(int64_t)1; }

static bool table_all_direct(int dim, int dtype, const LevelTable &lt, int64_t n) {
    LevelTable full = lt;
    full.level_begin = 0;
    full.level_end = lt.num_lods;
    BinPlan plan;
    make_plan(dim, dtype, full, kTile, plan, choose_acc_kib(dim, dtype, full, n), one_image_compact_rule(n));
    return plan.nbl == 0;
}

static uint64_t slots_per_sample(const BinPlan &plan) {
    uint64_t slots = 0;
    for (uint32_t q = 0; q < plan.nbl; ++q) {
        const BinLevel &bl = plan.lv[plan.blevel[q]];
        slots += bl.compact ? (plan.pairs == 4u ? 2u : 1u) : plan.pairs;
    }
    return slots;
}

static int front_tile(int L, int F, uint32_t nbl, int64_t n, size_t *shmem);

static void brick_levels_of_call(int dim, int dtype, const LevelTable &lt, int64_t n, const SortedBatch *sb, bool zero_table,
                                 bool grad_aligned, BrickPlan &brick, uint32_t &skip_mask) {
    brick.nlev = 0;
    skip_mask = 0u;
    if (dim != 3 || sb == nullptr) return;
    const int L = lt.num_lods, F = lt.feature_dim;
    const bool multi = bin_batch_samples(dim, dtype, lt, n) < n;
    const int kvec0 = (int)(16 / ((dtype == SHACIRA_F32 ? 4 : 2) * F));
    const int bopt = opt().bwd_brick;
    const bool wanted = bopt == 1 || (bopt < 0 && F == 2 && dtype == SHACIRA_F32);
    if (!wanted || multi || lt.stage_flags != 0 || !zero_table || n < SHACIRA_FX_MIN || n * L >= ((int64_t)1 << 31) ||
        table_all_direct(dim, dtype, lt, n) || (L % kvec0) != 0 || !grad_aligned)
        return;
    if (!make_brick_plan(lt, n, *sb, opt().bwd_brick_lo, opt().bwd_brick_hi, opt().bwd_brick_span,
                         (size_t)(opt().bwd_brick_fork == 2 ? 30 : 64) * 1024, brick)) {
        brick.nlev = 0;
        return;
    }
    for (uint32_t q = 0; q < brick.nlev; ++q) skip_mask |= 1u << brick.lv[q].level;
    BinPlan rest;
    make_plan(dim, dtype, lt, n, rest, choose_acc_kib(dim, dtype, lt, n), one_image_compact_rule(n), skip_mask, n);
    size_t sh0 = 0;
    if (rest.nbl == 0 || front_tile(L, F, rest.nbl, n, &sh0) <= 0) {
        skip_mask = 0u;
        brick.nlev = 0;
    }
}

static BinWorkspace carve(int dim, int dtype, const LevelTable &lt, int64_t n, void *ws, uint32_t skip_mask = 0u) {
    BinPlan plan;
    const int64_t nb = bin_batch_samples(dim, dtype, lt, n);
    make_plan(dim, dtype, lt, nb, plan, choose_acc_kib(dim, dtype, lt, n), one_image_compact_rule(n), skip_mask, n);
    const size_t item = item_unit_bytes(item_format(dim, dtype, lt, n), lt);
    size_t off = 0;
    auto take = [&](size_t bytes) { size_t o = off; off = align_up(off + bytes, 256); return o; };
    const bool no_stage = table_all_direct(dim, dtype, lt, n);
    const size_t o_gT = take(no_stage ? 0 : (size_t)level_pitch(n) * lt.num_lods * lt.feature_dim * sizeof(float));
    const size_t o_ctrl = take((size_t)(kTotalShards * kMaxBuckets + SHACIRA_MAX_LODS) * sizeof(uint32_t));
    const uint64_t pad_units = (uint64_t)plan.num_tiles * plan.total_buckets * (plan.pad - 1u);
    const size_t o_items = take(((size_t)nb * slots_per_sample(plan) + (size_t)pad_units) * item);
    const size_t o_base = take((size_t)(kMaxBuckets + 2) * sizeof(uint64_t));
    const size_t o_cur = take((size_t)(kMaxBuckets + 2) * sizeof(uint64_t));
    const size_t o_cnt = take((size_t)(nb / 128 + 8) * plan.total_buckets * sizeof(uint32_t));
    const size_t o_unit = take((size_t)(kMaxBuckets + 2) * sizeof(uint32_t));
    const uint64_t max_items_ws = (uint64_t)nb * plan.nbl * plan.pairs + pad_units;
    const size_t o_ub = take((size_t)(max_items_ws / plan.chunk_min + plan.total_buckets + 2) * sizeof(UnitDesc));
    const size_t o_wc = take(256);
    const size_t o_acc = take(dtype == SHACIRA_F16 ? (size_t)lt.table_rows * lt.feature_dim * sizeof(float) : 0);
    BinWorkspace w{};
    unsigned char *p = static_cast<unsigned char *>(ws);
    if (p) {
        w.gT = reinterpret_cast<float *>(p + o_gT);
        w.items = p + o_items;
        w.totals = reinterpret_cast<uint32_t *>(p + o_ctrl);
        w.gmax = w.totals + (size_t)kTotalShards * kMaxBuckets;
        w.base = reinterpret_cast<uint64_t *>(p + o_base);
        w.cursor = reinterpret_cast<unsigned long long *>(p + o_cur);
        w.cnt = reinterpret_cast<uint32_t *>(p + o_cnt);
        w.unit_first = reinterpret_cast<uint32_t *>(p + o_unit);
        w.unit_desc = reinterpret_cast<UnitDesc *>(p + o_ub);
        w.work_counter = reinterpret_cast<uint32_t *>(p + o_wc);
        w.acc32 = reinterpret_cast<float *>(p + o_acc);
    }
    w.bytes = off;
    return w;
}

static void resolve_call(int dim, int dtype, const LevelTable &lt, int64_t n, const SortedBatch *sb, bool zero_table,
                         bool grad_aligned, BrickPlan &brick, uint32_t &skip_mask) {
    const bool auto12 = opt().bwd_item12 < 0;
    if (auto12) {
        const bool brick_shape = sb != nullptr && dim == 3 && lt.feature_dim == 2 && dtype == SHACIRA_F32 &&
                                 lt.level_begin == 0 && lt.level_end == lt.num_lods && lt.stage_flags == 0 && zero_table &&
                                 opt().bwd_brick != 0;
        options_resolve_item12(brick_shape ? 1 : 0);
    }
    brick_levels_of_call(dim, dtype, lt, n, sb, zero_table, grad_aligned, brick, skip_mask);
    if (auto12 && brick.nlev == 0) options_resolve_item12(0);
}
static inline uint32_t carve_skip(int dtype, uint32_t skip_mask) { return dtype == SHACIRA_F32 ? skip_mask : 0u; }

size_t bin_workspace_bytes(int dim, int dtype, const LevelTable &lt, int64_t n) {
    return carve(dim, dtype, lt, n, nullptr).bytes;
}

size_t bin_workspace_bytes_planned(int dim, int dtype, const LevelTable &lt, int64_t n, bool whole, bool grad_aligned) {
    SortedBatch sb{};
    sample_plan_grid(dim, n, sb);
    BrickPlan brick;
    uint32_t skip_mask = 0;
    resolve_call(dim, dtype, lt, n, &sb, whole, grad_aligned, brick, skip_mask);
    return carve(dim, dtype, lt, n, nullptr, carve_skip(dtype, skip_mask)).bytes;
}

float *bin_acc32(int dim, int dtype, const LevelTable &lt, int64_t n, void *workspace) {
    return carve(dim, dtype, lt, n, workspace).acc32;
}

#define SHACIRA_CHECK_LAUNCH()                 \
    do {                                       \
        hipError_t e_ = hipGetLastError();     \
        if (e_ != hipSuccess) return e_;       \
    } while (0)
#define SHACIRA_CHECK(expr)                    \
    do {                                       \
        hipError_t e_ = (expr);                \
        if (e_ != hipSuccess) return e_;       \
    } while (0)

struct SideStream {
    hipStream_t stream = nullptr;
    hipEvent_t fork = nullptr, join = nullptr, staged = nullptr;
    hipEvent_t bfork = nullptr, bjoin = nullptr;
};
static hipError_t side_stream(SideStream **out) {
    static thread_local SideStream per_device[kMaxDevices];
    int dev = 0;
    SHACIRA_CHECK(hipGetDevice(&dev));
    if (dev < 0 || dev >= kMaxDevices) return hipErrorInvalidDevice;
    SideStream &ss = per_device[dev];
    if (!ss.stream) {
        hipStream_t st;
        hipEvent_t a, b, c, d, e;
        SHACIRA_CHECK(hipStreamCreateWithFlags(&st, hipStreamNonBlocking));
        SHACIRA_CHECK(hipEventCreateWithFlags(&a, hipEventDisableTiming));
        SHACIRA_CHECK(hipEventCreateWithFlags(&b, hipEventDisableTiming));
        SHACIRA_CHECK(hipEventCreateWithFlags(&c, hipEventDisableTiming));
        SHACIRA_CHECK(hipEventCreateWithFlags(&d, hipEventDisableTiming));
        SHACIRA_CHECK(hipEventCreateWithFlags(&e, hipEventDisableTiming));
        ss.fork = a;
        ss.join = b;
        ss.staged = c;
        ss.bfork = d;
        ss.bjoin = e;
        ss.stream = st;
    }
    *out = &ss;
    return hipSuccess;
}

static dim3 count_grid(const BinPlan &plan) {
    uint32_t shares = plan.num_tiles >= 1024 ? 1u : (1024u + plan.num_tiles - 1) / plan.num_tiles;
    if (shares > plan.nbl) shares = plan.nbl;
    return dim3(plan.num_tiles, shares < 1 ? 1 : shares);
}

static int front_tile(int L, int F, uint32_t nbl, int64_t n, size_t *shmem) {
    int ts = 512;
    for (;;) {
        const size_t bytes = (size_t)L * (ts + 2) * F * sizeof(float) + (size_t)nbl * kMaxLevelBuckets * sizeof(uint32_t);
        const bool enough = (n + ts - 1) / ts >= 512;
        if ((bytes <= (size_t)78 * 1024 && enough) || ts == 128) {
            *shmem = bytes;
            return bytes <= (size_t)156 * 1024 ? ts : 0;
        }
        ts /= 2;
    }
}

template <int DIM, int F>
static hipError_t run_bin(int dtype, const LevelTable &lt, const int32_t *first_idx, const float *coords,
                          const void *grad_out, float *acc, const BinWorkspace &w, int64_t n, hipStream_t s,
                          bool zero_table, __half *half_table, bool *converted, const SortedBatch *sb) {
    const int L = lt.num_lods;
    const int64_t NP = level_pitch(n);
    BinPlan whole;
    const int acc_kib = choose_acc_kib(DIM, dtype, lt, n);
    const bool oic = one_image_compact_rule(n);
    const int64_t nb = bin_batch_samples(DIM, dtype, lt, n);
    const bool multi = nb < n;
    const bool stage_all = (lt.stage_flags & SHACIRA_BWD_STAGE_ALL_LEVELS) != 0;
    const bool staged = (lt.stage_flags & SHACIRA_BWD_REUSE_STAGED) != 0;
    BrickPlan brick;
    uint32_t skip_mask = 0;
    brick_levels_of_call(DIM, dtype, lt, n, sb, zero_table, (reinterpret_cast<uintptr_t>(grad_out) & 15u) == 0, brick, skip_mask);
    make_plan(DIM, dtype, lt, n, whole, acc_kib, oic, skip_mask, n);
    const bool sorted = brick.nlev > 0;
    const float *cptr = sorted ? reinterpret_cast<const float *>(sb->sorted4) : coords;
    const int cstride = sorted ? 4 : DIM;
    int brick_mode = -1;
    SideStream *bss = nullptr;
    if (brick.nlev > 0) {
        brick_mode = opt().bwd_brick_fork;
        if (brick_mode > 0) SHACIRA_CHECK(side_stream(&bss));
    }
    auto launch_brick = [&](hipStream_t bs, hipEvent_t done = nullptr) -> hipError_t {
        if constexpr (DIM == 3) {
            const size_t img = (size_t)brick.rows_total * F * sizeof(double);
            const int hr = fx_headroom((uint64_t)kBrickUnit * 8u);
            const uint32_t groups = brick.groups_x * (uint32_t)(brick.nb[1] * brick.nb[2]);
            const uint32_t windows = (uint32_t)((n + kBrickUnit - 1) / kBrickUnit);
            if (done != nullptr)
                hipExtLaunchKernelGGL((brick_accumulate_kernel<F>), dim3(groups + windows), dim3(kBrickThreads), (uint32_t)img, bs,
                                      nullptr, done, 0u, lt, brick, first_idx, sb->sorted4, sb->block_start, (const float *)w.gT,
                                      NP, acc, (const uint32_t *)w.gmax, hr);
            else
                hipLaunchKernelGGL((brick_accumulate_kernel<F>), dim3(groups + windows), dim3(kBrickThreads), img, bs, lt, brick,
                                   first_idx, sb->sorted4, sb->block_start, w.gT, NP, acc, w.gmax, hr);
            return hipGetLastError();
        } else {
            (void)bs;
            return hipSuccess;
        }
    };
    auto fork_brick = [&]() -> hipError_t {
        SHACIRA_CHECK(hipEventRecord(bss->bfork, s));
        SHACIRA_CHECK(hipStreamWaitEvent(bss->stream, bss->bfork, 0));
        SHACIRA_CHECK(launch_brick(bss->stream));
        return hipEventRecord(bss->bjoin, bss->stream);
    };
    const bool need_T = whole.nbl > 0 || ((stage_all || staged) && !table_all_direct(DIM, dtype, lt, n));
    const bool use_fx = need_T && n >= SHACIRA_FX_MIN;
    const size_t esz = dtype == SHACIRA_F32 ? 4 : 2;
    const int kvec = (int)(16 / (esz * F));
    size_t front_shmem = 0;
    const int ts16 = front_tile(L, F, whole.nbl, n, &front_shmem);
    const bool t16 = ts16 > 0 && (L % kvec) == 0 && (reinterpret_cast<uintptr_t>(grad_out) & 15u) == 0;
    const bool front_counts = need_T && !staged && !multi && t16 && whole.nbl > 0;
    const bool direct_half = half_table != nullptr && half_items(dtype, lt) && !multi && !stage_all && !staged &&
                             whole.nbl > 0 && lt.level_begin == 0 && lt.level_end == L;
    const int64_t fork_work = n * lt.num_lods * lt.feature_dim;
    const int64_t fork_min = DIM == 3 ? ((int64_t)7 << 21) : ((int64_t)1 << 23);
    const bool fork = whole.nbl > 0 && whole.ngroups > 0 && !multi && opt().bwd_fork != 0 && fork_work >= fork_min &&
                      brick_mode <= 0;
    bool any_hashed = false;
    for (uint32_t q = 0; q < whole.nbl; ++q) any_hashed = any_hashed || lt.dense[whole.blevel[q]] == 0;
    const bool selective = zero_table && !multi && any_hashed && opt().bwd_selective_zero != 0;
    SideStream *ss = nullptr;
    hipStream_t zs = s;
    if (fork) {
        SHACIRA_CHECK(side_stream(&ss));
        SHACIRA_CHECK(hipEventRecord(ss->fork, s));
        SHACIRA_CHECK(hipStreamWaitEvent(ss->stream, ss->fork, 0));
        zs = ss->stream;
    }
    const bool need_words = whole.nbl > 0 || (!staged && use_fx);
    const uint32_t words = (uint32_t)kTotalShards * kMaxBuckets + ((!staged && use_fx) ? SHACIRA_MAX_LODS : 0);
    bool words_done = false;
    if (zero_table) {
        if (!selective) {
            SHACIRA_CHECK(zero_fill_async(acc, (int64_t)lt.table_rows * lt.feature_dim, zs));
        } else {
            words_done = need_words && zs == s;
            hipLaunchKernelGGL(zero_unowned_rows_kernel, dim3(256, (uint32_t)L + (words_done ? 1u : 0u)), dim3(256), 0, zs, acc,
                               first_idx, lt, whole, w.totals, words);
            SHACIRA_CHECK_LAUNCH();
        }
    }
    if (need_words && !words_done) {
        hipLaunchKernelGGL(zero_words_kernel, dim3(32), dim3(256), 0, s, w.totals, words);
        SHACIRA_CHECK_LAUNCH();
    }
    if (need_T && !staged) {
        const int t_lb = stage_all ? 0 : lt.level_begin, t_le = stage_all ? L : lt.level_end;
        if (t16) {
            const int64_t tiles = (n + ts16 - 1) / ts16;
            int ts_log2 = 7;
            while ((1 << ts_log2) < ts16) ++ts_log2;
            int rounds = (int)((tiles + 511) / 512);
            const int cps16 = TileOf<DIM>::value / ts16;
            if (whole.pad > 1u && front_counts) rounds = (rounds + cps16 - 1) / cps16 * cps16;
            const uint32_t blocks = (uint32_t)((tiles + rounds - 1) / rounds);
#define SHACIRA_FRONT(TT, GM, CN)                                                                                         \
            hipLaunchKernelGGL((front16_kernel<DIM, TT, F, GM, CN>), dim3(blocks), dim3(kFrontThreads), front_shmem, s, lt, \
                               whole, static_cast<const TT *>(grad_out), w.gT, coords, w.totals, w.cnt, n, NP, t_lb, t_le, ts_log2, \
                               rounds, GM ? w.gmax : nullptr, (uint32_t)cps16)
#define SHACIRA_FRONT_SORTED(TT)                                                                                          \
            hipLaunchKernelGGL((front16_kernel<DIM, TT, F, true, true, true>), dim3(blocks), dim3(kFrontThreads), front_shmem, s, lt, \
                               whole, static_cast<const TT *>(grad_out), w.gT, coords, w.totals, w.cnt, n, NP, t_lb, t_le, ts_log2, \
                               rounds, w.gmax, (uint32_t)cps16, sb->sorted4)
            if (sorted) {
                if (dtype == SHACIRA_F32) SHACIRA_FRONT_SORTED(float);
                else SHACIRA_FRONT_SORTED(__half);
            } else if (dtype == SHACIRA_F32) {
                if (use_fx && front_counts) SHACIRA_FRONT(float, true, true);
                else if (use_fx) SHACIRA_FRONT(float, true, false);
                else if (front_counts) SHACIRA_FRONT(float, false, true);
                else SHACIRA_FRONT(float, false, false);
            } else {
                if (use_fx && front_counts) SHACIRA_FRONT(__half, true, true);
                else if (use_fx) SHACIRA_FRONT(__half, true, false);
                else if (front_counts) SHACIRA_FRONT(__half, false, true);
                else SHACIRA_FRONT(__half, false, false);
            }
#undef SHACIRA_FRONT
#undef SHACIRA_FRONT_SORTED
        } else {
            const uint32_t blocks = (uint32_t)((n + 255) / 256);
            const size_t shmem = (size_t)256 * (L + 1) * F * sizeof(float);
            if (dtype == SHACIRA_F32 && use_fx)
                hipLaunchKernelGGL((transpose_grad_kernel<float, F, true>), dim3(blocks), dim3(256), shmem, s,
                                   static_cast<const float *>(grad_out), w.gT, n, NP, L, t_lb, t_le, w.gmax);
            else if (dtype == SHACIRA_F32)
                hipLaunchKernelGGL((transpose_grad_kernel<float, F, false>), dim3(blocks), dim3(256), shmem, s,
                                   static_cast<const float *>(grad_out), w.gT, n, NP, L, t_lb, t_le, nullptr);
            else if (use_fx)
                hipLaunchKernelGGL((transpose_grad_kernel<__half, F, true>), dim3(blocks), dim3(256), shmem, s,
                                   static_cast<const __half *>(grad_out), w.gT, n, NP, L, t_lb, t_le, w.gmax);
            else
                hipLaunchKernelGGL((transpose_grad_kernel<__half, F, false>), dim3(blocks), dim3(256), shmem, s,
                                   static_cast<const __half *>(grad_out), w.gT, n, NP, L, t_lb, t_le, nullptr);
        }
        SHACIRA_CHECK_LAUNCH();
    }
    if (fork) {
        SHACIRA_CHECK(hipEventRecord(ss->staged, s));
        SHACIRA_CHECK(hipStreamWaitEvent(ss->stream, ss->staged, 0));
    }
    if (brick_mode == 1) SHACIRA_CHECK(fork_brick());
    if (whole.ngroups > 0) {
        const BinPlan &plan = whole;
        uint32_t bpg = (plan.ngroups > 1 ? 256u : 512u) / plan.ngroups;
        const uint32_t need = (uint32_t)((n + 2047) / 2048);
        if (bpg > need) bpg = need;
        if (bpg < 1) bpg = 1;
        const size_t acc_bytes = (size_t)plan.BR * F * sizeof(double);
        const dim3 grid(bpg, plan.ngroups);
        const int headroom = fx_headroom(((uint64_t)n / bpg + kConsumeThreads) * (1u << DIM));
        const uint32_t *gm = (need_T && use_fx) ? w.gmax : nullptr;
        if (need_T)
            hipLaunchKernelGGL((direct_accumulate_kernel<DIM, F, float, true, true>), grid, dim3(kConsumeThreads),
                               acc_bytes, zs, lt, plan, first_idx, cptr, w.gT, acc, n, NP, gm, headroom, cstride);
        else if (dtype == SHACIRA_F32)
            hipLaunchKernelGGL((direct_accumulate_kernel<DIM, F, float, false, true>), grid, dim3(kConsumeThreads),
                               acc_bytes, zs, lt, plan, first_idx, coords, static_cast<const float *>(grad_out), acc, n,
                               NP, gm, headroom);
        else
            hipLaunchKernelGGL((direct_accumulate_kernel<DIM, F, __half, false, true>), grid, dim3(kConsumeThreads),
                               acc_bytes, zs, lt, plan, first_idx, coords, static_cast<const __half *>(grad_out), acc, n,
                               NP, gm, headroom);
        SHACIRA_CHECK_LAUNCH();
    }
    if (fork) SHACIRA_CHECK(hipEventRecord(ss->join, ss->stream));
    if (whole.nbl == 0) return hipSuccess;
    constexpr int NPAIR = 1 << (DIM - 1);
    const int fmt = item_format(DIM, dtype, lt, n);
    const bool half = fmt == 1;
    auto stage_bytes = [&](const BinPlan &pl) -> size_t {
        const size_t isz = fmt == 2 ? sizeof(Item12) : half ? sizeof(typename ItemSel<F, true>::type) : sizeof(Item<F>);
        const int split = half ? ScatterSplit<typename ItemSel<F, true>::type>::value : ScatterSplit<Item<F>>::value;
        const size_t units = split == 1 ? (size_t)pl.stage_cap : (size_t)TileOf<DIM>::value * NPAIR / split;
        return units * (isz + 1);
    };
#ifdef SCATTER_LEVEL_FAST
#define SCATTER_GRID(pl) dim3((pl).nbl, (pl).num_tiles)
#else
#define SCATTER_GRID(pl) dim3((pl).num_tiles, (pl).nbl)
#endif
    bool first_batch = true;
    for (int64_t s0 = 0; s0 < n; s0 += nb) {
        const int64_t hi = (s0 + nb < n) ? (s0 + nb) : n;
        BinPlan plan;
        make_plan(DIM, dtype, lt, hi - s0, plan, acc_kib, oic, skip_mask, n);
        if (!first_batch) {
            hipLaunchKernelGGL(zero_words_kernel, dim3(32), dim3(256), 0, s, w.totals, (uint32_t)kTotalShards * kMaxBuckets);
            SHACIRA_CHECK_LAUNCH();
        }
        const bool fused_now = front_counts && first_batch;
        if (!fused_now) {
            hipLaunchKernelGGL((bin_count_levels_kernel<DIM>), count_grid(plan), dim3(kBinThreads), 0, s, lt, plan, coords,
                               w.totals, w.cnt, s0, hi);
            SHACIRA_CHECK_LAUNCH();
        }
        first_batch = false;
        hipLaunchKernelGGL(bin_scan_buckets_kernel, dim3(1), dim3(1024), 0, s, w.totals, w.base, w.unit_first, w.unit_desc,
                           plan.total_buckets, plan, w.work_counter, w.cursor, use_fx ? w.gmax : nullptr);
        SHACIRA_CHECK_LAUNCH();
        float *zacc = selective ? acc : nullptr;
        const uint32_t cps = fused_now ? (uint32_t)(TileOf<DIM>::value / ts16) : 1u;
        const uint32_t cnt_rows = fused_now ? (uint32_t)((n + ts16 - 1) / ts16) : plan.num_tiles;
        bool fork_signalled = false;
        if (fmt == 2) {
            if constexpr (DIM == 3 && F == 2) {
                hipStreamCaptureStatus cap = hipStreamCaptureStatusNone;
                if (brick_mode == 2 && opt().bwd_ext_fork != 0 && hipStreamIsCapturing(s, &cap) == hipSuccess &&
                    cap == hipStreamCaptureStatusNone) {
                    hipExtLaunchKernelGGL((bin_scatter_kernel<DIM, F, 2>), SCATTER_GRID(plan),
                                          dim3(ScatterThreads<DIM, F, 2>::value), (uint32_t)stage_bytes(plan), s, nullptr,
                                          bss->bfork, 0u, lt, plan, cptr, (const float *)w.gT, w.cursor, (const uint32_t *)w.cnt, cps, cnt_rows,
                                          reinterpret_cast<Item12 *>(w.items), s0, hi, NP, zacc, first_idx,
                                          (const uint32_t *)w.unit_first, cstride);
                    fork_signalled = true;
                } else {
                    hipLaunchKernelGGL((bin_scatter_kernel<DIM, F, 2>), SCATTER_GRID(plan), dim3(ScatterThreads<DIM, F, 2>::value),
                                       stage_bytes(plan), s, lt, plan, cptr, w.gT, w.cursor, w.cnt, cps, cnt_rows,
                                       reinterpret_cast<Item12 *>(w.items), s0, hi, NP, zacc, first_idx, w.unit_first, cstride);
                }
            }
        } else if (half)
            hipLaunchKernelGGL((bin_scatter_kernel<DIM, F, true>), SCATTER_GRID(plan), dim3(ScatterThreads<DIM, F, 1>::value),
                               stage_bytes(plan), s, lt, plan, cptr, w.gT, w.cursor, w.cnt, cps, cnt_rows,
                               reinterpret_cast<typename ItemSel<F, true>::type *>(w.items), s0, hi, NP, zacc, first_idx,
                               w.unit_first, cstride);
        else if (use_fx)
            hipLaunchKernelGGL((bin_scatter_kernel<DIM, F, false>), SCATTER_GRID(plan), dim3(ScatterThreads<DIM, F, 0>::value),
                               stage_bytes(plan), s, lt, plan, cptr, w.gT, w.cursor, w.cnt, cps, cnt_rows,
                               reinterpret_cast<Item<F> *>(w.items), s0, hi, NP, zacc, first_idx, w.unit_first, cstride);
        else
            hipLaunchKernelGGL((bin_scatter_kernel<DIM, F, false, false>), SCATTER_GRID(plan), dim3(ScatterThreads<DIM, F, 0>::value),
                               stage_bytes(plan), s, lt, plan, cptr, w.gT, w.cursor, w.cnt, cps, cnt_rows,
                               reinterpret_cast<Item<F> *>(w.items), s0, hi, NP, zacc, first_idx, w.unit_first, cstride);
        SHACIRA_CHECK_LAUNCH();
        if (fork) SHACIRA_CHECK(hipStreamWaitEvent(s, ss->join, 0));
        if (brick_mode == 2) {
            if (fork_signalled) {
                SHACIRA_CHECK(hipStreamWaitEvent(bss->stream, bss->bfork, 0));
                SHACIRA_CHECK(launch_brick(bss->stream, bss->bjoin));
            } else {
                SHACIRA_CHECK(fork_brick());
            }
        }
        const uint64_t max_items = (uint64_t)(hi - s0) * plan.nbl * NPAIR +
                                   (uint64_t)plan.num_tiles * plan.total_buckets * (plan.pad - 1u);
        uint32_t grid_units = (uint32_t)(max_items / plan.chunk_min) + plan.total_buckets + 1;
        const size_t acc_bytes = (size_t)plan.BR * F * sizeof(double);
        uint32_t *wc = (opt().bwd_persistent != 0 && n >= SHACIRA_PERSIST_MIN) ? w.work_counter : nullptr;
        if (wc != nullptr && grid_units > 512u) grid_units = 512u;
        const int headroom = use_fx ? fx_headroom((uint64_t)plan.chunk + 1) : -1;
        const int fa = multi ? 1 : 0;
        __half *hout = direct_half ? half_table : nullptr;
        if (fmt == 2) {
            if constexpr (DIM == 3 && F == 2)
                hipLaunchKernelGGL((bin_consume_kernel<F, true, 2>), dim3(grid_units), dim3(kConsumeThreads), acc_bytes, s, lt,
                                   plan, first_idx, w.unit_first, w.unit_desc, reinterpret_cast<const Item12 *>(w.items), acc,
                                   fa, headroom, wc);
        } else if (half && use_fx)
            hipLaunchKernelGGL((bin_consume_kernel<F, true, true>), dim3(grid_units), dim3(kConsumeThreads), acc_bytes, s,
                               lt, plan, first_idx, w.unit_first, w.unit_desc,
                               reinterpret_cast<const typename ItemSel<F, true>::type *>(w.items), acc, fa, headroom, wc, hout);
        else if (half)
            hipLaunchKernelGGL((bin_consume_kernel<F, false, true>), dim3(grid_units), dim3(kConsumeThreads), acc_bytes, s,
                               lt, plan, first_idx, w.unit_first, w.unit_desc,
                               reinterpret_cast<const typename ItemSel<F, true>::type *>(w.items), acc, fa, headroom, wc, hout);
        else if (use_fx)
            hipLaunchKernelGGL((bin_consume_kernel<F, true, false>), dim3(grid_units), dim3(kConsumeThreads), acc_bytes, s, lt,
                               plan, first_idx, w.unit_first, w.unit_desc,
                               reinterpret_cast<const Item<F> *>(w.items), acc, fa, headroom, wc);
        else if (!half)
            hipLaunchKernelGGL((bin_consume_kernel<F, false, false>), dim3(grid_units), dim3(kConsumeThreads), acc_bytes, s, lt,
                               plan, first_idx, w.unit_first, w.unit_desc,
                               reinterpret_cast<const Item<F> *>(w.items), acc, fa, headroom, wc);
        SHACIRA_CHECK_LAUNCH();
    }
    if (brick_mode == 0) SHACIRA_CHECK(launch_brick(s));
    if (brick_mode > 0) SHACIRA_CHECK(hipStreamWaitEvent(s, bss->bjoin, 0));
    if (direct_half) {
        hipLaunchKernelGGL(f32_to_f16_skip_kernel, dim3(128, (uint32_t)L), dim3(256), 0, s, acc, half_table, first_idx, lt,
                           whole, w.unit_first, F);
        SHACIRA_CHECK_LAUNCH();
        if (converted != nullptr) *converted = true;
    }
    return hipSuccess;
}

template <class ItemT> static constexpr size_t stage_max(size_t tile_units) {
    constexpr size_t split = ScatterSplit<ItemT>::value;
    constexpr size_t padu = split != 1 ? 0 : sizeof(ItemT) == 16 ? SHACIRA_RUN_ALIGN / 16 - 1 : sizeof(ItemT) == 12 ? SHACIRA_RUN_ALIGN / 4 - 1
                            : (SHACIRA_PAD_HALF && sizeof(ItemT) == 8) ? SHACIRA_RUN_ALIGN / 8 - 1 : 0;
    return (tile_units / split + (size_t)kMaxLevelBuckets * padu) * (sizeof(ItemT) + 1);
}

hipError_t bin_backward(int dim, int dtype, const LevelTable &lt, const int32_t *first_idx, const float *coords,
                        const void *grad_out, float *acc, void *workspace, int64_t n, hipStream_t s, bool zero_table,
                        void *half_table, bool *converted, const SortedBatch *sb) {
    if (converted != nullptr) *converted = false;
    __half *ht = (dtype == SHACIRA_F16) ? static_cast<__half *>(half_table) : nullptr;
    BrickPlan brick;
    uint32_t skip_mask = 0;
    resolve_call(dim, dtype, lt, n, sb, zero_table, (reinterpret_cast<uintptr_t>(grad_out) & 15u) == 0, brick, skip_mask);
    const BinWorkspace w = carve(dim, dtype, lt, n, workspace, carve_skip(dtype, skip_mask));
    static PerDeviceOnce once;
    const hipError_t attr_err = once.run([]() -> hipError_t {
        hipError_t attr_err = hipSuccess;
        auto set = [&attr_err](const void *fn, size_t bytes) {
            if (bytes <= 64 * 1024 || bytes > 160 * 1024) return;
            hipError_t e = hipFuncSetAttribute(fn, hipFuncAttributeMaxDynamicSharedMemorySize, (int)bytes);
            if (e != hipSuccess) attr_err = e;
        };
#define SHACIRA_T_ATTR(TT, FF)                                                                           \
        set(reinterpret_cast<const void *>(&transpose_grad_kernel<TT, FF, true>), 140 * 1024);          \
        set(reinterpret_cast<const void *>(&transpose_grad_kernel<TT, FF, false>), 140 * 1024);         \
        set(reinterpret_cast<const void *>(&front16_kernel<2, TT, FF, true, true>), 156 * 1024);        \
        set(reinterpret_cast<const void *>(&front16_kernel<2, TT, FF, true, false>), 156 * 1024);       \
        set(reinterpret_cast<const void *>(&front16_kernel<2, TT, FF, false, true>), 156 * 1024);       \
        set(reinterpret_cast<const void *>(&front16_kernel<2, TT, FF, false, false>), 156 * 1024);      \
        set(reinterpret_cast<const void *>(&front16_kernel<3, TT, FF, true, true>), 156 * 1024);        \
        set(reinterpret_cast<const void *>(&front16_kernel<3, TT, FF, true, false>), 156 * 1024);       \
        set(reinterpret_cast<const void *>(&front16_kernel<3, TT, FF, false, true>), 156 * 1024);       \
        set(reinterpret_cast<const void *>(&front16_kernel<3, TT, FF, false, false>), 156 * 1024);      \
        set(reinterpret_cast<const void *>(&front16_kernel<3, TT, FF, true, true, true>), 156 * 1024);
        SHACIRA_T_ATTR(float, 2) SHACIRA_T_ATTR(float, 4) SHACIRA_T_ATTR(__half, 2) SHACIRA_T_ATTR(__half, 4)
#undef SHACIRA_T_ATTR
#define SHACIRA_DIRECT_ATTR(D, FF)                                                                              \
        set(reinterpret_cast<const void *>(&direct_accumulate_kernel<D, FF, float, true, true>), 16384 * sizeof(double));   \
        set(reinterpret_cast<const void *>(&direct_accumulate_kernel<D, FF, float, false, true>), 16384 * sizeof(double));  \
        set(reinterpret_cast<const void *>(&direct_accumulate_kernel<D, FF, __half, false, true>), 16384 * sizeof(double));
        SHACIRA_DIRECT_ATTR(2, 2) SHACIRA_DIRECT_ATTR(2, 4) SHACIRA_DIRECT_ATTR(3, 2) SHACIRA_DIRECT_ATTR(3, 4)
#undef SHACIRA_DIRECT_ATTR
        set(reinterpret_cast<const void *>(&bin_consume_kernel<2, true, 2>), 16384 * sizeof(double));
        set(reinterpret_cast<const void *>(&bin_scatter_kernel<3, 2, 2>), stage_max<Item12>(TileOf<3>::value << 2));
        set(reinterpret_cast<const void *>(&bin_consume_kernel<2, true, false>), 16384 * sizeof(double));
        set(reinterpret_cast<const void *>(&bin_consume_kernel<4, true, false>), 16384 * sizeof(double));
        set(reinterpret_cast<const void *>(&bin_consume_kernel<2, false, false>), 16384 * sizeof(double));
        set(reinterpret_cast<const void *>(&bin_consume_kernel<4, false, false>), 16384 * sizeof(double));
        set(reinterpret_cast<const void *>(&bin_consume_kernel<2, true, true>), 16384 * sizeof(double));
        set(reinterpret_cast<const void *>(&bin_consume_kernel<2, false, true>), 16384 * sizeof(double));
        set(reinterpret_cast<const void *>(&bin_consume_kernel<4, true, true>), 16384 * sizeof(double));
        set(reinterpret_cast<const void *>(&bin_consume_kernel<4, false, true>), 16384 * sizeof(double));
        set(reinterpret_cast<const void *>(&bin_scatter_kernel<2, 2, true>), stage_max<ItemH>(TileOf<2>::value << 1));
        set(reinterpret_cast<const void *>(&bin_scatter_kernel<3, 2, true>), stage_max<ItemH>(TileOf<3>::value << 2));
        set(reinterpret_cast<const void *>(&bin_scatter_kernel<2, 4, true>), stage_max<typename ItemSel<4, true>::type>(TileOf<2>::value << (2 - 1)));
        set(reinterpret_cast<const void *>(&bin_scatter_kernel<3, 4, true>), stage_max<typename ItemSel<4, true>::type>(TileOf<3>::value << (3 - 1)));
        set(reinterpret_cast<const void *>(&bin_scatter_kernel<2, 2, false>), stage_max<Item<2>>(TileOf<2>::value << (2 - 1)));
        set(reinterpret_cast<const void *>(&bin_scatter_kernel<2, 4, false>), stage_max<Item<4>>(TileOf<2>::value << (2 - 1)));
        set(reinterpret_cast<const void *>(&bin_scatter_kernel<3, 2, false>), stage_max<Item<2>>(TileOf<3>::value << (3 - 1)));
        set(reinterpret_cast<const void *>(&bin_scatter_kernel<3, 4, false>), stage_max<Item<4>>(TileOf<3>::value << (3 - 1)));
        set(reinterpret_cast<const void *>(&bin_scatter_kernel<2, 2, false, false>), stage_max<Item<2>>(TileOf<2>::value << (2 - 1)));
        set(reinterpret_cast<const void *>(&bin_scatter_kernel<2, 4, false, false>), stage_max<Item<4>>(TileOf<2>::value << (2 - 1)));
        set(reinterpret_cast<const void *>(&bin_scatter_kernel<3, 2, false, false>), stage_max<Item<2>>(TileOf<3>::value << (3 - 1)));
        set(reinterpret_cast<const void *>(&bin_scatter_kernel<3, 4, false, false>), stage_max<Item<4>>(TileOf<3>::value << (3 - 1)));
        return attr_err;
    });
    if (attr_err != hipSuccess) return attr_err;
    if (dim == 3) {
        return lt.feature_dim == 2 ? run_bin<3, 2>(dtype, lt, first_idx, coords, grad_out, acc, w, n, s, zero_table, ht, converted, sb)
                                   : run_bin<3, 4>(dtype, lt, first_idx, coords, grad_out, acc, w, n, s, zero_table, ht, converted, sb);
    }
    return lt.feature_dim == 2 ? run_bin<2, 2>(dtype, lt, first_idx, coords, grad_out, acc, w, n, s, zero_table, ht, converted, nullptr)
                               : run_bin<2, 4>(dtype, lt, first_idx, coords, grad_out, acc, w, n, s, zero_table, ht, converted, nullptr);
}

}

#ifdef CONSUME_TRACE
extern "C" __attribute__((visibility("default"))) int shacira_debug_consume_trace(unsigned long long *host, unsigned int cap,
                                                                                   unsigned int *count) {
    unsigned int n = 0;
    if (hipMemcpyFromSymbol(&n, HIP_SYMBOL(shacira::g_consume_trace_n), sizeof(n)) != hipSuccess) return 1;
    *count = n;
    if (n > cap) n = cap;
    if (n > 16384u) n = 16384u;
    if (n && hipMemcpyFromSymbol(host, HIP_SYMBOL(shacira::g_consume_trace), (size_t)n * 8 * sizeof(unsigned long long)) != hipSuccess)
        return 2;
    unsigned int zero = 0;
    if (hipMemcpyToSymbol(HIP_SYMBOL(shacira::g_consume_trace_n), &zero, sizeof(zero)) != hipSuccess) return 3;
    return 0;
}
#endif
```

### shacira_amd/csrc/internal.h

```cpp
#pragma once

#include <atomic>
#include <mutex>

#include "hashgrid_device.h"

namespace shacira {

constexpr int kMaxDevices = 64;
struct PerDeviceOnce {
    std::once_flag flag[kMaxDevices];
    hipError_t err[kMaxDevices] = {};
    template <typename Fn> hipError_t run(Fn &&fn) {
        int dev = 0;
        hipError_t e = hipGetDevice(&dev);
        if (e != hipSuccess) return e;
        if (dev < 0 || dev >= kMaxDevices) return hipErrorInvalidDevice;
        std::call_once(flag[dev], [&] { err[dev] = fn(); });
        return err[dev];
    }
};

size_t hashgrid_forward_workspace(int dim, int dtype, const LevelTable &lt, int64_t n);
hipError_t hashgrid_forward_dispatch(int dim, int dtype, const LevelTable &lt, const int32_t *first_idx,
                                     const float *coords, const void *table, void *feats, void *workspace, int64_t n,
                                     hipStream_t s, void *plan = nullptr, bool plan_ready = false);
hipError_t hashgrid_forward_levels_staged(int dim, int dtype, const LevelTable &lt, const int32_t *first_idx,
                                          const float *coords, const void *table, void *staged, int64_t n,
                                          hipStream_t s);
hipError_t hashgrid_forward_rows(int dim, int dtype, const LevelTable &lt, const int32_t *first_idx, const float *sorted4,
                                 const void *table, const void *staged, void *feats, int64_t n, int lc, hipStream_t s);
bool tiled_supported(int dim, int dtype, const LevelTable &lt, int64_t n);
size_t tiled_forward_workspace(int dim, int dtype, const LevelTable &lt, int64_t n);
hipError_t tiled_forward(int dim, int dtype, const LevelTable &lt, const int32_t *first_idx, const float *coords,
                         const void *table, void *feats, void *workspace, int64_t n, hipStream_t s, void *plan = nullptr,
                         bool plan_ready = false);
struct SortedBatch {
    const float4 *sorted4;
    const uint32_t *block_start;
    uint32_t num_blocks;
    int32_t nb[3];
};
size_t sample_plan_bytes(int dim, int64_t n);
size_t sample_plan_scratch_bytes(int dim, int64_t n);
hipError_t sample_plan_build(int dim, const float *coords, int64_t n, void *plan, void *scratch, hipStream_t s);
void sample_plan_view(int dim, int64_t n, const void *plan, SortedBatch &out);
void sample_plan_grid(int dim, int64_t n, SortedBatch &out);
hipError_t hashgrid_debug_corners(int dim, const LevelTable &lt, const float *coords, int64_t n, int32_t *idx, float *w,
                                  hipStream_t s);
hipError_t hashgrid_coord_grad_dispatch(int dim, int dtype, const LevelTable &lt, const int32_t *first_idx,
                                        const float *coords, const void *table, const void *grad_out,
                                        float *grad_coords, int64_t n, hipStream_t s, const void *plan);
hipError_t zero_fill_async(float *p, int64_t n, hipStream_t s);
size_t hashgrid_backward_workspace(int dim, int dtype, const LevelTable &lt, int64_t n);
size_t hashgrid_backward_workspace_planned(int dim, int dtype, const LevelTable &lt, int64_t n, bool grad_aligned);
hipError_t hashgrid_backward_dispatch(int dim, int dtype, const LevelTable &lt, const int32_t *first_idx,
                                      const float *coords, const void *grad_out, void *grad_table, void *workspace,
                                      size_t workspace_bytes, int64_t n, hipStream_t s, const void *plan = nullptr);

struct TriplaneArgs {
    const float *plane[3 * SHACIRA_TRIPLANE_MAX_LODS];
    float *grad[3 * SHACIRA_TRIPLANE_MAX_LODS];
    int64_t hwc_off[3 * SHACIRA_TRIPLANE_MAX_LODS];
    int32_t side[SHACIRA_TRIPLANE_MAX_LODS];
    int32_t num_lods;
    int32_t fdim;
};
struct TriBwdPlan {
    int32_t nb, nbins;
    int32_t sort_side;
    int32_t cells;
    int32_t sum;
    int32_t win[SHACIRA_TRIPLANE_MAX_LODS];
};
constexpr int kTriDefaultHwc = 1;
size_t triplane_forward_workspace(const TriplaneArgs &a, int64_t n);
hipError_t triplane_forward_dispatch(TriplaneArgs a, const float *coords, int sum, float *feats, void *workspace,
                                     int64_t n, hipStream_t s);
void triplane_backward_plan(const TriplaneArgs &a, int sum, TriBwdPlan &bp);
size_t triplane_backward_workspace(const TriplaneArgs &a, int sum, int64_t n);
hipError_t triplane_backward_dispatch(const TriplaneArgs &a, const float *coords, const float *grad_out, int sum,
                                      bool planes, float *grad_coords, void *workspace, int64_t n, hipStream_t s);

struct DecodeArgs {
    const float *latent, *div, *matrix, *colscale, *shift;
    float clampw;
    float *decoded;
    const float *grad_decoded;
    float *grad_latent, *grad_matrix, *grad_colscale, *grad_shift;
    double *partials;
    int64_t rows;
    const float *uniforms;
    float temperature;
    int diff_sampling;
    const float *temperature_dev;
};
struct EntropyArgs {
    const float *latent, *noise, *params, *grad_total;
    int num_layers;
    float *total_bits, *grad_latent, *grad_params;
    double *partials;
    int64_t rows;
};
struct LatentMlpArgs {
    int num_layers;
    const int32_t *widths;
    const float *latent, *uniforms, *div, *params;
    float temperature;
    int diff_sampling, act, final_act;
    float clampw;
    float *decoded;
    const float *grad_decoded;
    float *grad_latent, *grad_params;
    double *partials;
    int64_t rows;
};
bool latent_mlp_supported(int num_layers, const int32_t *widths);
size_t latent_mlp_workspace_bytes(int num_layers, const int32_t *widths);
hipError_t latent_mlp_dispatch(bool bwd, const LatentMlpArgs &a, hipStream_t s);

size_t latent_workspace_bytes();
bool latent_decode_supported(int ld, int f);
hipError_t latent_decode_dispatch(bool bwd, int ld, int f, const DecodeArgs &a, hipStream_t s);
hipError_t latent_decode_levels_dispatch(bool bwd, int ld, int f, int levels, const int64_t *offsets,
                                         const DecodeArgs &a, hipStream_t s);
bool latent_multi_supported(int ld, int f, int K);
hipError_t latent_multi_dispatch(bool bwd, int ld, int f, bool dft, const float *latent, const float *alpha, int K,
                                 const float *uniforms, float temperature, int straight_through, int diff_sampling,
                                 const float *div, const float *scale, const float *dftm, const float *shift,
                                 float clampw, int64_t rows, float *decoded, const float *grad_decoded,
                                 float *grad_latent, float *grad_alpha, float *grad_scale, float *grad_shift,
                                 double *partials, hipStream_t s);
bool entropy_supported(int ld);
hipError_t entropy_dispatch(bool bwd, int ld, const EntropyArgs &a, hipStream_t s);

bool symbols_supported(int ld);
hipError_t symbol_range_launch(const float *latent, int64_t rows, int ld, int32_t *minmax, hipStream_t s);
hipError_t symbol_histogram_launch(const float *latent, int64_t rows, int ld, const int32_t *minmax, int nbins,
                                   uint64_t *counts, hipStream_t s);
size_t rc_encode_bound(int64_t n);
int rc_encode(const int32_t *sym, int64_t n, const uint32_t *freq, int nsym, uint8_t *out, size_t cap, size_t *len);
int rc_decode(const uint8_t *in, size_t len, const uint32_t *freq, int nsym, int64_t n, int32_t *sym);

hipError_t pack_integrate_launch(bool bwd, int64_t R, int C, const float *feats, const float *tau,
                                 const int64_t *pack_start, float *ray_feats, float *weights, const float *g_ray,
                                 const float *g_w, float *g_feats, float *g_tau, hipStream_t s);
hipError_t pack_sum_launch(bool broadcast, int64_t R, int C, const float *in, const int64_t *pack_start, float *out,
                           hipStream_t s);
hipError_t raymarch_ray_launch(bool emit, int64_t num_rays, int ns, const float *origins, const float *dirs,
                               float dist_min, float dist_max, const float *lin, const float *jitter,
                               const uint8_t *occ, int level, int32_t *counts, const int64_t *offsets, int64_t *ridx,
                               float *samples, float *depth, float *deltas, uint8_t *boundary, int64_t capacity,
                               hipStream_t s);
hipError_t raytrace_dense_launch(bool emit, int64_t num_rays, const float *origins, const float *dirs,
                                 const uint8_t *occ, int level, int32_t *counts, const int64_t *offsets, int32_t *ridx,
                                 int32_t *pidx, float *depth, hipStream_t s);

hipError_t stream_probe_launch(int kind, const void *a, void *b, size_t bytes, uint32_t *sink, hipStream_t s);

hipError_t adam_step_launch(float *p, float *g, float *m, float *v, int64_t n, float lr, float b1, float b2, float eps,
                            float wd, int step, const int32_t *step_dev, int zero_grad, hipStream_t s);

hipError_t adam_multi_launch(int count, float *const *p, float *const *g, float *const *m, float *const *v,
                             const int64_t *n, const float *lr, const float *wd, float b1, float b2, float eps,
                             int step, const int32_t *step_dev, int zero_grad, hipStream_t s);

constexpr int kMlpMaxBlocks = 512;
constexpr int kMlpNarrowMaxBlocks = 512;
bool mlp_supported(int in, int h, int nh, int out);
int mlp_num_params(int in, int h, int nh, int out);
size_t mlp_workspace_bytes(int in, int h, int nh, int out);
hipError_t mlp_dispatch(bool bwd, int in, int h, int nh, int out, int64_t N, const float *x, const float *params,
                        float *y, const float *gy, float *gx, float *gparams, double *partials, hipStream_t s);

struct Options {
    int fwd_variant = -1;
    int bwd_variant = -1;
    int mlp_variant = -1;
    int bwd_compact = 1;
    int bwd_selective_zero = 1;
    int bwd_persistent = 1;
    int bwd_fork = 1;
    int bwd_item12 = -1;
    int bwd_run_pad = 1;
    int bin_acc_kib = 0;
    int bin_batch_mib = 1536;
    int tiled = -1;
    int tiled_lc_fwd = -1;
    int bwd_brick = -1;
    int bwd_brick_lo = -1;
    int bwd_brick_hi = -1;
    int bwd_brick_fork = 2;
    int bwd_brick_span = 0;
    int bwd_ext_fork = 1;
    int coord_variant = -1;
    int fwd_direct = -1;
    int triplane_layout = -1;
};
const Options &opt();
void options_snapshot();
void options_resolve_item12(int value);

}
```

Measured before the change: 1.414 billion.

## Fold bucket scan into scatter kernel and split brick work across streams

Removes the single-block bucket-scan kernel launch. The scan now runs in an extra slot of the scatter grid, and each scatter block computes its own per-bucket global base from the shard totals plus precomputed per-level region offsets, so it no longer needs a serial scan. The cursor is zeroed together with the totals, and the selective-zero test reads the totals directly. Brick work can also be split into low and high parts, launched earlier on a side stream behind a front event, with RAII join guards. This trades a serialized launch and dependency for redundant totals reads in every block, larger reserved item regions per level, and more complex stream synchronization.

```diff
diff --git a/shacira_amd/csrc/api.hip b/shacira_amd/csrc/api.hip
--- a/shacira_amd/csrc/api.hip
+++ b/shacira_amd/csrc/api.hip
@@ -32,6 +32,7 @@
     {"bwd_brick_hi", &Options::bwd_brick_hi, -1, SHACIRA_MAX_LODS, {-1}},
     {"bwd_brick_fork", &Options::bwd_brick_fork, 0, 2, {2}},
     {"bwd_brick_span", &Options::bwd_brick_span, 0, 64, {0}},
+    {"bwd_brick_split", &Options::bwd_brick_split, -1, 6, {-1}},
     {"fwd_direct", &Options::fwd_direct, -1, 1, {-1}},
     {"bwd_ext_fork", &Options::bwd_ext_fork, 0, 1, {1}},
     {"coord_variant", &Options::coord_variant, -1, 8, {-1}},
diff --git a/shacira_amd/csrc/bwd_bin_front.h b/shacira_amd/csrc/bwd_bin_front.h
--- a/shacira_amd/csrc/bwd_bin_front.h
+++ b/shacira_amd/csrc/bwd_bin_front.h
@@ -279,38 +279,54 @@
     }
 }
 
-__global__ __launch_bounds__(1024) void bin_scan_buckets_kernel(const uint32_t *__restrict__ totals,
-                                                                uint64_t *__restrict__ base,
-                                                                uint32_t *__restrict__ unit_first,
-                                                                UnitDesc *__restrict__ unit_desc, uint32_t nb,
-                                                                BinPlan plan,
-                                                                uint32_t *__restrict__ work_counter,
-                                                                unsigned long long *__restrict__ cursor,
-                                                                const uint32_t *__restrict__ gmax) {
-    __shared__ uint64_t s_items[kMaxBuckets + 2];
-    __shared__ uint32_t s_units[kMaxBuckets + 2];
-    __shared__ uint64_t s_wave_items[16];
-    __shared__ uint32_t s_wave_units[16];
+constexpr size_t kScanLdsBytes = (size_t)(kMaxBuckets + 2) * (sizeof(uint64_t) + sizeof(uint32_t)) +
+                                 16 * (sizeof(uint64_t) + sizeof(uint32_t)) + SHACIRA_MAX_LODS * (sizeof(uint64_t) + 2 * sizeof(uint32_t));
+template <int KT>
+__device__ __forceinline__ void bin_scan_buckets(unsigned char *s_raw, const uint32_t *__restrict__ totals,
+                                                 uint64_t *__restrict__ base, uint32_t *__restrict__ unit_first,
+                                                 UnitDesc *__restrict__ unit_desc, const BinPlan &plan,
+                                                 uint32_t *__restrict__ work_counter, const uint32_t *__restrict__ gmax) {
+    static_assert(KT % 64 == 0 && KT <= 1024 && kMaxBuckets % KT == 0, "whole waves, at most 16 of them");
+    constexpr int PER = kMaxBuckets / KT;
+    uint64_t *s_items = reinterpret_cast<uint64_t *>(s_raw);
+    uint32_t *s_units = reinterpret_cast<uint32_t *>(s_items + kMaxBuckets + 2);
+    uint64_t *s_wave_items = reinterpret_cast<uint64_t *>(s_units + kMaxBuckets + 2);
+    uint64_t *s_region = s_wave_items + 16;
+    uint32_t *s_wave_units = reinterpret_cast<uint32_t *>(s_region + SHACIRA_MAX_LODS);
+    uint32_t *s_bstart = s_wave_units + 16;
+    uint32_t *s_blevel = s_bstart + SHACIRA_MAX_LODS;
+    const uint32_t nb = plan.total_buckets;
     const uint32_t t = threadIdx.x, lane = t & 63, wave = t >> 6;
     if (t == 0) work_counter[0] = 0;
-    uint64_t c[2];
-    uint32_t u[2], lv_of[2], ck[2];
-#pragma unroll
-    for (int k = 0; k < 2; ++k) {
-        const uint32_t b = 2 * t + k;
+#pragma unroll
+    for (uint32_t q = 0; q < SHACIRA_MAX_LODS; ++q)
+        if (t == q) {
+            s_bstart[q] = plan.bstart[q];
+            s_blevel[q] = plan.blevel[q];
+            s_region[q] = plan.level_base[q];
+        }
+    uint64_t c[PER];
+    uint32_t u[PER];
+    const uint32_t ck = plan.chunk;
+#pragma unroll
+    for (int k = 0; k < PER; ++k) {
+        const uint32_t b = PER * t + k;
         c[k] = 0u;
-        if (b < nb)
+        if (b < nb) {
+#pragma unroll 4
             for (int sh = 0; sh < kTotalShards; ++sh) c[k] += totals[(size_t)sh * kMaxBuckets + b];
-        uint32_t lvl = plan.blevel[0];
-#pragma unroll
-        for (uint32_t q = 1; q < SHACIRA_MAX_LODS; ++q)
-            if (q < plan.nbl && plan.bstart[q] <= b) lvl = plan.blevel[q];
-        lv_of[k] = lvl;
-        ck[k] = plan.chunk;
-        u[k] = (c[k] >> 32) ? (uint32_t)((c[k] + ck[k] - 1) / ck[k]) : (c[k] ? ((uint32_t)c[k] - 1u) / ck[k] + 1u : 0u);
-    }
-    uint64_t ci = c[0] + c[1];
-    uint32_t ui = u[0] + u[1];
+        }
+        u[k] = (c[k] >> 32) ? (uint32_t)((c[k] + ck - 1) / ck) : (c[k] ? ((uint32_t)c[k] - 1u) / ck + 1u : 0u);
+    }
+    uint64_t csum = 0;
+    uint32_t usum = 0;
+#pragma unroll
+    for (int k = 0; k < PER; ++k) {
+        csum += c[k];
+        usum += u[k];
+    }
+    uint64_t ci = csum;
+    uint32_t ui = usum;
 #pragma unroll
     for (int off = 1; off < 64; off <<= 1) {
         const uint64_t nc = __shfl_up(ci, off, 64);
@@ -322,33 +338,41 @@
     uint64_t wc = 0;
     uint32_t wu = 0;
     for (uint32_t w = 0; w < wave; ++w) { wc += s_wave_items[w]; wu += s_wave_units[w]; }
-    const uint64_t ex_items = wc + ci - (c[0] + c[1]);
-    const uint32_t ex_units = wu + ui - (u[0] + u[1]);
-    s_items[2 * t] = ex_items;
-    s_items[2 * t + 1] = ex_items + c[0];
-    s_units[2 * t] = ex_units;
-    s_units[2 * t + 1] = ex_units + u[0];
-    if (t == 1023) {
-        s_items[kMaxBuckets] = ex_items + c[0] + c[1];
-        s_units[kMaxBuckets] = ex_units + u[0] + u[1];
-    }
-    __syncthreads();
-    for (uint32_t b = t; b <= nb; b += 1024) {
-        base[b] = s_items[b];
-        cursor[b] = s_items[b];
-        unit_first[b] = s_units[b];
-    }
-#pragma unroll
-    for (int k = 0; k < 2; ++k) {
-        const uint32_t b = 2 * t + k;
+    uint64_t ex_items = wc + ci - csum;
+    uint32_t ex_units = wu + ui - usum;
+#pragma unroll
+    for (int k = 0; k < PER; ++k) {
+        s_items[PER * t + k] = ex_items;
+        s_units[PER * t + k] = ex_units;
+        ex_items += c[k];
+        ex_units += u[k];
+    }
+    if (t == KT - 1) {
+        s_items[kMaxBuckets] = ex_items;
+        s_units[kMaxBuckets] = ex_units;
+    }
+    __syncthreads();
+    if (t == 0) {
+        const uint32_t ql = plan.nbl - 1u;
+        base[nb] = s_region[ql] + (s_items[nb] - s_items[s_bstart[ql]]);
+        unit_first[nb] = s_units[nb];
+    }
+#pragma unroll
+    for (int k = 0; k < PER; ++k) {
+        const uint32_t b = PER * t + k;
         if (b < nb) {
-            const uint32_t lvl = lv_of[k];
+            uint32_t ql = 0;
+            for (uint32_t q = 1; q < plan.nbl; ++q) ql = s_bstart[q] <= b ? q : ql;
+            const uint32_t lvl = s_blevel[ql];
+            const uint64_t first = s_region[ql] + (s_items[b] - s_items[s_bstart[ql]]);
+            base[b] = first;
+            unit_first[b] = s_units[b];
             const uint32_t gm = (gmax != nullptr && u[k] > 0) ? gmax[lvl] : 0u;
             for (uint32_t q = 0; q < u[k]; ++q) {
                 UnitDesc d;
-                d.begin = s_items[b] + (uint64_t)q * ck[k];
-                const uint64_t bucket_end = s_items[b] + c[k];
-                d.end = (d.begin + ck[k] < bucket_end) ? (d.begin + ck[k]) : bucket_end;
+                d.begin = first + (uint64_t)q * ck;
+                const uint64_t bucket_end = first + c[k];
+                d.end = (d.begin + ck < bucket_end) ? (d.begin + ck) : bucket_end;
                 d.bucket = b;
                 d.level = lvl;
                 d.single = u[k] == 1 ? 1u : 0u;
@@ -421,9 +445,11 @@
 __global__ __launch_bounds__(256) void zero_unowned_rows_kernel(float *__restrict__ acc,
                                                                 const int32_t *__restrict__ first_idx, LevelTable lt,
                                                                 BinPlan plan, uint32_t *__restrict__ words,
-                                                                uint32_t nwords) {
+                                                                uint32_t nwords, uint32_t *__restrict__ words2,
+                                                                uint32_t nwords2) {
     if ((int)blockIdx.y == lt.num_lods) {
         for (uint32_t i = blockIdx.x * 256 + threadIdx.x; i < nwords; i += gridDim.x * 256) words[i] = 0u;
+        for (uint32_t i = blockIdx.x * 256 + threadIdx.x; i < nwords2; i += gridDim.x * 256) words2[i] = 0u;
         return;
     }
     const int l = blockIdx.y, F = lt.feature_dim;
@@ -440,8 +466,10 @@
     for (int64_t e = hole_hi * F + t0; e < end * F; e += stride) acc[e] = 0.0f;
 }
 
-__global__ __launch_bounds__(256) void zero_words_kernel(uint32_t *__restrict__ p, uint32_t n) {
+__global__ __launch_bounds__(256) void zero_words_kernel(uint32_t *__restrict__ p, uint32_t n, uint32_t *__restrict__ p2,
+                                                         uint32_t n2) {
     for (uint32_t i = blockIdx.x * 256 + threadIdx.x; i < n; i += gridDim.x * 256) p[i] = 0u;
+    for (uint32_t i = blockIdx.x * 256 + threadIdx.x; i < n2; i += gridDim.x * 256) p2[i] = 0u;
 }
 
 template <int F> __device__ __forceinline__ void rotate_features(const float (&a)[F], int rot, float (&r)[F]) {
diff --git a/shacira_amd/csrc/bwd_bin_passes.h b/shacira_amd/csrc/bwd_bin_passes.h
--- a/shacira_amd/csrc/bwd_bin_passes.h
+++ b/shacira_amd/csrc/bwd_bin_passes.h
@@ -20,8 +20,13 @@
                                                                   int64_t sample0, int64_t N, int64_t gpitch,
                                                                   float *__restrict__ zero_acc,
                                                                   const int32_t *__restrict__ first_idx,
-                                                                  const uint32_t *__restrict__ unit_first,
-                                                                  int cstride = DIM) {
+                                                                  const uint32_t *__restrict__ totals,
+                                                                  int cstride,
+                                                                  uint64_t *__restrict__ scan_base,
+                                                                  uint32_t *__restrict__ scan_unit_first,
+                                                                  UnitDesc *__restrict__ scan_unit_desc,
+                                                                  uint32_t *__restrict__ work_counter,
+                                                                  const uint32_t *__restrict__ gmax) {
     typedef typename ItemSel<F, FMT>::type ItemT;
     constexpr bool H = FMT == 1;
     constexpr bool P12 = FMT == 2;
@@ -41,13 +46,22 @@
     __shared__ uint64_t s_gbase[kMaxLevelBuckets];
 
 #ifdef SCATTER_LEVEL_FAST
-    const uint32_t tile = blockIdx.y, bi = blockIdx.x;
+    const uint32_t slot = blockIdx.y, bi = blockIdx.x;
 #else
-    const uint32_t tile = blockIdx.x, bi = blockIdx.y;
+    const uint32_t slot = blockIdx.x, bi = blockIdx.y;
 #endif
+    if (slot == 0u) {
+        if (bi == 0u)
+            bin_scan_buckets<kThreads>(s_raw, totals, scan_base, scan_unit_first, scan_unit_desc, plan, work_counter, gmax);
+        return;
+    }
+    const uint32_t tile = slot - 1u;
     const uint32_t lvl = plan.blevel[bi];
     const BinLevel bl = plan.lv[lvl];
-    if (threadIdx.x < kMaxLevelBuckets) s_hist[threadIdx.x] = 0;
+    if (threadIdx.x < kMaxLevelBuckets) {
+        s_hist[threadIdx.x] = 0;
+        s_gbase[threadIdx.x] = 0;
+    }
     __syncthreads();
     const int32_t res = lt.res[lvl];
     const float hi = lt.hi[lvl];
@@ -78,6 +92,15 @@
 #pragma unroll
             for (int j = 0; j < F; ++j) graw[u][j] = gp[j];
         }
+    }
+    constexpr int kTotWords = kTotalShards * kMaxLevelBuckets / kThreads;
+    static_assert(kTotWords * kThreads == kTotalShards * kMaxLevelBuckets, "whole words per thread");
+    uint32_t traw[kTotWords];
+#pragma unroll
+    for (int j = 0; j < kTotWords; ++j) {
+        const uint32_t wd = threadIdx.x + (uint32_t)j * kThreads;
+        const uint32_t b = wd % kMaxLevelBuckets;
+        traw[j] = totals[(size_t)(wd / kMaxLevelBuckets) * kMaxBuckets + bl.bucket0 + (b < bl.nb ? b : 0u)];
     }
     const bool reserver = threadIdx.x >= 64 && threadIdx.x - 64 < bl.nb;
     unsigned long long run_base = 0ull;
@@ -88,10 +111,15 @@
         for (uint32_t k = 0; k < cps && tile * cps + k < cnt_rows; ++k) c += row[(size_t)k * plan.total_buckets];
         c = (c + plan.pad - 1u) & ~(plan.pad - 1u);
 #ifdef ABL_NO_CURSOR
-        if (c) run_base = cursor[gb] + (unsigned long long)tile * c;
+        if (c) run_base = (unsigned long long)tile * c;
 #else
         if (c) run_base = atomicAdd(&cursor[gb], (unsigned long long)c);
 #endif
+    }
+#pragma unroll
+    for (int j = 0; j < kTotWords; ++j) {
+        const uint32_t b = (threadIdx.x + (uint32_t)j * kThreads) % kMaxLevelBuckets;
+        if (b < bl.nb && traw[j]) atomicAdd(reinterpret_cast<unsigned long long *>(&s_gbase[b]), (unsigned long long)traw[j]);
     }
 #pragma unroll
     for (int u = 0; u < SPT; ++u) {
@@ -148,6 +176,23 @@
         }
     }
     lds_barrier();
+    if (threadIdx.x >= 64 && threadIdx.x < 128) {
+        const uint32_t lane = threadIdx.x - 64;
+        const bool h0 = 2 * lane < bl.nb, h1 = 2 * lane + 1 < bl.nb;
+        uint64_t incl = (h0 ? s_gbase[2 * lane] : 0u) + (h1 ? s_gbase[2 * lane + 1] : 0u);
+#pragma unroll
+        for (int off = 1; off < 64; off <<= 1) {
+            const uint64_t nbr = __shfl_up(incl, off, 64);
+            if (lane >= (uint32_t)off) incl += nbr;
+        }
+        asm volatile("" ::: "memory");
+        if (h1) {
+            const uint64_t t1 = s_gbase[2 * lane + 1];
+            s_gbase[2 * lane + 1] = incl - t1;
+            incl -= t1;
+        }
+        if (h0) s_gbase[2 * lane] = incl - s_gbase[2 * lane];
+    }
     if (threadIdx.x < 64) {
         const uint32_t lane = threadIdx.x;
         const uint32_t pm = plan.pad - 1u;
@@ -307,7 +352,7 @@
         }
     }
     if (wi == 0) {
-        if (reserver) s_gbase[threadIdx.x - 64] = run_base;
+        if (reserver) s_gbase[threadIdx.x - 64] += plan.level_base[bi] + run_base;
         __syncthreads();
     } else {
         lds_barrier();
@@ -324,7 +369,9 @@
     if (zero_acc != nullptr && !dense) {
         for (uint32_t b = tile; b < bl.nb; b += plan.num_tiles) {
             const uint32_t gb = bl.bucket0 + b;
-            if (unit_first[gb + 1] - unit_first[gb] == 1u) continue;
+            uint64_t tot = 0;
+            for (int sh = 0; sh < kTotalShards; ++sh) tot += totals[(size_t)sh * kMaxBuckets + gb];
+            if (tot != 0u && tot <= (uint64_t)plan.chunk) continue;
             const uint32_t row0 = b * bl.rows_pb;
             const uint32_t nrows = (bl.used - row0 < bl.rows_pb) ? (bl.used - row0) : bl.rows_pb;
             float *dst = zero_acc + ((int64_t)first_idx[lvl] + row0) * F;
diff --git a/shacira_amd/csrc/bwd_bin_types.h b/shacira_amd/csrc/bwd_bin_types.h
--- a/shacira_amd/csrc/bwd_bin_types.h
+++ b/shacira_amd/csrc/bwd_bin_types.h
@@ -66,6 +66,7 @@
     uint32_t blevel[SHACIRA_MAX_LODS];
     uint32_t bstart[SHACIRA_MAX_LODS];
     uint32_t bnb[SHACIRA_MAX_LODS];
+    uint64_t level_base[SHACIRA_MAX_LODS];
     uint32_t ngroups;
     uint32_t gmask[SHACIRA_MAX_LODS];
     uint32_t grows[SHACIRA_MAX_LODS];
diff --git a/shacira_amd/csrc/hashgrid_bwd_bin.hip b/shacira_amd/csrc/hashgrid_bwd_bin.hip
--- a/shacira_amd/csrc/hashgrid_bwd_bin.hip
+++ b/shacira_amd/csrc/hashgrid_bwd_bin.hip
@@ -287,6 +287,15 @@
         }
     }
     plan.chunk_min = plan.chunk;
+    uint64_t region = 0;
+    for (uint32_t q = 0; q < (uint32_t)SHACIRA_MAX_LODS; ++q) {
+        plan.level_base[q] = region;
+        if (q >= plan.nbl) continue;
+        const BinLevel &bl = plan.lv[plan.blevel[q]];
+        const uint64_t per_sample = bl.compact ? (plan.pairs == 4u ? 2u : 1u) : plan.pairs;
+        const uint64_t worst = (uint64_t)n_batch * per_sample + (uint64_t)plan.num_tiles * bl.nb * (plan.pad - 1u);
+        region += worst / plan.pad * plan.pad;
+    }
 }
 
 static inline bool half_items(int dtype, const LevelTable &lt) {
@@ -464,6 +473,16 @@
     hipStream_t stream = nullptr;
     hipEvent_t fork = nullptr, join = nullptr, staged = nullptr;
     hipEvent_t bfork = nullptr, bjoin = nullptr;
+    hipEvent_t bfront = nullptr;
+};
+struct JoinGuard {
+    hipStream_t main = nullptr, side = nullptr;
+    hipEvent_t ev = nullptr;
+    void arm(hipStream_t main_, hipStream_t side_, hipEvent_t ev_) { main = main_; side = side_; ev = ev_; }
+    void disarm() { ev = nullptr; }
+    ~JoinGuard() {
+        if (ev != nullptr && hipEventRecord(ev, side) == hipSuccess) (void)hipStreamWaitEvent(main, ev, 0);
+    }
 };
 static hipError_t side_stream(SideStream **out) {
     static thread_local SideStream per_device[kMaxDevices];
@@ -473,18 +492,20 @@
     SideStream &ss = per_device[dev];
     if (!ss.stream) {
         hipStream_t st;
-        hipEvent_t a, b, c, d, e;
+        hipEvent_t a, b, c, d, e, f;
         SHACIRA_CHECK(hipStreamCreateWithFlags(&st, hipStreamNonBlocking));
         SHACIRA_CHECK(hipEventCreateWithFlags(&a, hipEventDisableTiming));
         SHACIRA_CHECK(hipEventCreateWithFlags(&b, hipEventDisableTiming));
         SHACIRA_CHECK(hipEventCreateWithFlags(&c, hipEventDisableTiming));
         SHACIRA_CHECK(hipEventCreateWithFlags(&d, hipEventDisableTiming));
         SHACIRA_CHECK(hipEventCreateWithFlags(&e, hipEventDisableTiming));
+        SHACIRA_CHECK(hipEventCreateWithFlags(&f, hipEventDisableTiming));
         ss.fork = a;
         ss.join = b;
         ss.staged = c;
         ss.bfork = d;
         ss.bjoin = e;
+        ss.bfront = f;
         ss.stream = st;
     }
     *out = &ss;
@@ -508,6 +529,18 @@
         }
         ts /= 2;
     }
+}
+
+constexpr double kBrickSplitReuse = 25.0;
+static uint32_t brick_split_rule(const BrickPlan &bp, int64_t n) {
+    if (bp.num_blocks == 0) return 0;
+    const double unit_samples = (double)n / (double)bp.num_blocks * (double)bp.span;
+    uint32_t k = 0;
+    for (; k < bp.nlev; ++k) {
+        const double rows = (double)bp.lv[k].w[0] * bp.lv[k].w[1] * bp.lv[k].w[2];
+        if (8.0 * unit_samples < kBrickSplitReuse * rows) break;
+    }
+    return k;
 }
 
 template <int DIM, int F>
@@ -532,11 +565,29 @@
     const int cstride = sorted ? 4 : DIM;
     int brick_mode = -1;
     SideStream *bss = nullptr;
+    JoinGuard brick_guard;
     if (brick.nlev > 0) {
         brick_mode = opt().bwd_brick_fork;
         if (brick_mode > 0) SHACIRA_CHECK(side_stream(&bss));
     }
-    auto launch_brick = [&](hipStream_t bs, hipEvent_t done = nullptr) -> hipError_t {
+    BrickPlan brick_low, brick_high;
+    brick_low.nlev = 0;
+    brick_high.nlev = 0;
+    uint32_t brick_split = 0;
+    if (brick_mode == 2 && opt().bwd_brick_lo < 0) {
+        const int sopt = opt().bwd_brick_split;
+        uint32_t k = sopt >= 0 ? (uint32_t)sopt : brick_split_rule(brick, n);
+        if (k > brick.nlev) k = brick.nlev;
+        const size_t budget = (size_t)30 * 1024;
+        const int l0 = (int)brick.level0, l1 = l0 + (int)k, l2 = l0 + (int)brick.nlev;
+        bool ok = k > 0;
+        if (ok) ok = make_brick_plan(lt, n, *sb, l0, l1, (int)brick.span, budget, brick_low) && brick_low.nlev == k;
+        if (ok && l1 < l2)
+            ok = make_brick_plan(lt, n, *sb, l1, l2, (int)brick.span, budget, brick_high) && brick_high.nlev == brick.nlev - k;
+        if (ok) brick_split = k;
+        else brick_high.nlev = 0;
+    }
+    auto launch_brick = [&](const BrickPlan &brick, hipStream_t bs, hipEvent_t done = nullptr) -> hipError_t {
         if constexpr (DIM == 3) {
             const size_t img = (size_t)brick.rows_total * F * sizeof(double);
             const int hr = fx_headroom((uint64_t)kBrickUnit * 8u);
@@ -551,16 +602,24 @@
                                    first_idx, sb->sorted4, sb->block_start, w.gT, NP, acc, w.gmax, hr);
             return hipGetLastError();
         } else {
+            (void)brick;
             (void)bs;
+            (void)done;
             return hipSuccess;
         }
     };
     auto fork_brick = [&]() -> hipError_t {
         SHACIRA_CHECK(hipEventRecord(bss->bfork, s));
         SHACIRA_CHECK(hipStreamWaitEvent(bss->stream, bss->bfork, 0));
-        SHACIRA_CHECK(launch_brick(bss->stream));
+        brick_guard.arm(s, bss->stream, bss->bjoin);
+        SHACIRA_CHECK(launch_brick(brick, bss->stream));
         return hipEventRecord(bss->bjoin, bss->stream);
     };
+    bool ext_ok = false;
+    if (brick_mode == 2 && opt().bwd_ext_fork != 0) {
+        hipStreamCaptureStatus cap = hipStreamCaptureStatusNone;
+        ext_ok = hipStreamIsCapturing(s, &cap) == hipSuccess && cap == hipStreamCaptureStatusNone;
+    }
     const bool need_T = whole.nbl > 0 || ((stage_all || staged) && !table_all_direct(DIM, dtype, lt, n));
     const bool use_fx = need_T && n >= SHACIRA_FX_MIN;
     const size_t esz = dtype == SHACIRA_F32 ? 4 : 2;
@@ -579,15 +638,19 @@
     for (uint32_t q = 0; q < whole.nbl; ++q) any_hashed = any_hashed || lt.dense[whole.blevel[q]] == 0;
     const bool selective = zero_table && !multi && any_hashed && opt().bwd_selective_zero != 0;
     SideStream *ss = nullptr;
+    JoinGuard fork_guard;
     hipStream_t zs = s;
     if (fork) {
         SHACIRA_CHECK(side_stream(&ss));
         SHACIRA_CHECK(hipEventRecord(ss->fork, s));
         SHACIRA_CHECK(hipStreamWaitEvent(ss->stream, ss->fork, 0));
+        fork_guard.arm(s, ss->stream, ss->join);
         zs = ss->stream;
     }
     const bool need_words = whole.nbl > 0 || (!staged && use_fx);
     const uint32_t words = (uint32_t)kTotalShards * kMaxBuckets + ((!staged && use_fx) ? SHACIRA_MAX_LODS : 0);
+    uint32_t *const cursor_words = reinterpret_cast<uint32_t *>(w.cursor);
+    constexpr uint32_t kCursorWords = (uint32_t)(kMaxBuckets + 2) * 2u;
     bool words_done = false;
     if (zero_table) {
         if (!selective) {
@@ -595,12 +658,12 @@
         } else {
             words_done = need_words && zs == s;
             hipLaunchKernelGGL(zero_unowned_rows_kernel, dim3(256, (uint32_t)L + (words_done ? 1u : 0u)), dim3(256), 0, zs, acc,
-                               first_idx, lt, whole, w.totals, words);
+                               first_idx, lt, whole, w.totals, words, cursor_words, kCursorWords);
             SHACIRA_CHECK_LAUNCH();
         }
     }
     if (need_words && !words_done) {
-        hipLaunchKernelGGL(zero_words_kernel, dim3(32), dim3(256), 0, s, w.totals, words);
+        hipLaunchKernelGGL(zero_words_kernel, dim3(32), dim3(256), 0, s, w.totals, words, cursor_words, kCursorWords);
         SHACIRA_CHECK_LAUNCH();
     }
     if (need_T && !staged) {
@@ -621,7 +684,15 @@
             hipLaunchKernelGGL((front16_kernel<DIM, TT, F, true, true, true>), dim3(blocks), dim3(kFrontThreads), front_shmem, s, lt, \
                                whole, static_cast<const TT *>(grad_out), w.gT, coords, w.totals, w.cnt, n, NP, t_lb, t_le, ts_log2, \
                                rounds, w.gmax, (uint32_t)cps16, sb->sorted4)
-            if (sorted) {
+#define SHACIRA_FRONT_SORTED_EXT(TT)                                                                                      \
+            hipExtLaunchKernelGGL((front16_kernel<DIM, TT, F, true, true, true>), dim3(blocks), dim3(kFrontThreads),       \
+                                  (uint32_t)front_shmem, s, nullptr, bss->bfront, 0u, lt, whole, static_cast<const TT *>(grad_out), \
+                                  w.gT, coords, w.totals, w.cnt, n, NP, t_lb, t_le, ts_log2, rounds, w.gmax, (uint32_t)cps16,    \
+                                  (const float4 *)sb->sorted4)
+            if (sorted && brick_split > 0 && ext_ok) {
+                if (dtype == SHACIRA_F32) SHACIRA_FRONT_SORTED_EXT(float);
+                else SHACIRA_FRONT_SORTED_EXT(__half);
+            } else if (sorted) {
                 if (dtype == SHACIRA_F32) SHACIRA_FRONT_SORTED(float);
                 else SHACIRA_FRONT_SORTED(__half);
             } else if (dtype == SHACIRA_F32) {
@@ -637,6 +708,7 @@
             }
 #undef SHACIRA_FRONT
 #undef SHACIRA_FRONT_SORTED
+#undef SHACIRA_FRONT_SORTED_EXT
         } else {
             const uint32_t blocks = (uint32_t)((n + 255) / 256);
             const size_t shmem = (size_t)256 * (L + 1) * F * sizeof(float);
@@ -660,6 +732,17 @@
         SHACIRA_CHECK(hipStreamWaitEvent(ss->stream, ss->staged, 0));
     }
     if (brick_mode == 1) SHACIRA_CHECK(fork_brick());
+    if (brick_split > 0) {
+        if (!ext_ok) SHACIRA_CHECK(hipEventRecord(bss->bfront, s));
+        SHACIRA_CHECK(hipStreamWaitEvent(bss->stream, bss->bfront, 0));
+        brick_guard.arm(s, bss->stream, bss->bjoin);
+        if (brick_high.nlev == 0 && ext_ok) {
+            SHACIRA_CHECK(launch_brick(brick_low, bss->stream, bss->bjoin));
+        } else {
+            SHACIRA_CHECK(launch_brick(brick_low, bss->stream));
+            if (brick_high.nlev == 0) SHACIRA_CHECK(hipEventRecord(bss->bjoin, bss->stream));
+        }
+    }
     if (whole.ngroups > 0) {
         const BinPlan &plan = whole;
         uint32_t bpg = (plan.ngroups > 1 ? 256u : 512u) / plan.ngroups;
@@ -692,12 +775,13 @@
         const size_t isz = fmt == 2 ? sizeof(Item12) : half ? sizeof(typename ItemSel<F, true>::type) : sizeof(Item<F>);
         const int split = half ? ScatterSplit<typename ItemSel<F, true>::type>::value : ScatterSplit<Item<F>>::value;
         const size_t units = split == 1 ? (size_t)pl.stage_cap : (size_t)TileOf<DIM>::value * NPAIR / split;
-        return units * (isz + 1);
+        const size_t bytes = units * (isz + 1);
+        return bytes > kScanLdsBytes ? bytes : kScanLdsBytes;
     };
 #ifdef SCATTER_LEVEL_FAST
-#define SCATTER_GRID(pl) dim3((pl).nbl, (pl).num_tiles)
+#define SCATTER_GRID(pl) dim3((pl).nbl, (pl).num_tiles + 1u)
 #else
-#define SCATTER_GRID(pl) dim3((pl).num_tiles, (pl).nbl)
+#define SCATTER_GRID(pl) dim3((pl).num_tiles + 1u, (pl).nbl)
 #endif
     bool first_batch = true;
     for (int64_t s0 = 0; s0 < n; s0 += nb) {
@@ -705,7 +789,8 @@
         BinPlan plan;
         make_plan(DIM, dtype, lt, hi - s0, plan, acc_kib, oic, skip_mask, n);
         if (!first_batch) {
-            hipLaunchKernelGGL(zero_words_kernel, dim3(32), dim3(256), 0, s, w.totals, (uint32_t)kTotalShards * kMaxBuckets);
+            hipLaunchKernelGGL(zero_words_kernel, dim3(32), dim3(256), 0, s, w.totals, (uint32_t)kTotalShards * kMaxBuckets,
+                               cursor_words, kCursorWords);
             SHACIRA_CHECK_LAUNCH();
         }
         const bool fused_now = front_counts && first_batch;
@@ -715,51 +800,58 @@
             SHACIRA_CHECK_LAUNCH();
         }
         first_batch = false;
-        hipLaunchKernelGGL(bin_scan_buckets_kernel, dim3(1), dim3(1024), 0, s, w.totals, w.base, w.unit_first, w.unit_desc,
-                           plan.total_buckets, plan, w.work_counter, w.cursor, use_fx ? w.gmax : nullptr);
-        SHACIRA_CHECK_LAUNCH();
+        const uint32_t *scan_gmax = use_fx ? w.gmax : nullptr;
         float *zacc = selective ? acc : nullptr;
         const uint32_t cps = fused_now ? (uint32_t)(TileOf<DIM>::value / ts16) : 1u;
         const uint32_t cnt_rows = fused_now ? (uint32_t)((n + ts16 - 1) / ts16) : plan.num_tiles;
         bool fork_signalled = false;
         if (fmt == 2) {
             if constexpr (DIM == 3 && F == 2) {
-                hipStreamCaptureStatus cap = hipStreamCaptureStatusNone;
-                if (brick_mode == 2 && opt().bwd_ext_fork != 0 && hipStreamIsCapturing(s, &cap) == hipSuccess &&
-                    cap == hipStreamCaptureStatusNone) {
+                if (ext_ok && (brick_split == 0 || brick_high.nlev > 0)) {
                     hipExtLaunchKernelGGL((bin_scatter_kernel<DIM, F, 2>), SCATTER_GRID(plan),
                                           dim3(ScatterThreads<DIM, F, 2>::value), (uint32_t)stage_bytes(plan), s, nullptr,
                                           bss->bfork, 0u, lt, plan, cptr, (const float *)w.gT, w.cursor, (const uint32_t *)w.cnt, cps, cnt_rows,
                                           reinterpret_cast<Item12 *>(w.items), s0, hi, NP, zacc, first_idx,
-                                          (const uint32_t *)w.unit_first, cstride);
+                                          (const uint32_t *)w.totals, cstride, w.base, w.unit_first, w.unit_desc, w.work_counter,
+                                          scan_gmax);
                     fork_signalled = true;
                 } else {
                     hipLaunchKernelGGL((bin_scatter_kernel<DIM, F, 2>), SCATTER_GRID(plan), dim3(ScatterThreads<DIM, F, 2>::value),
                                        stage_bytes(plan), s, lt, plan, cptr, w.gT, w.cursor, w.cnt, cps, cnt_rows,
-                                       reinterpret_cast<Item12 *>(w.items), s0, hi, NP, zacc, first_idx, w.unit_first, cstride);
+                                       reinterpret_cast<Item12 *>(w.items), s0, hi, NP, zacc, first_idx, w.totals, cstride, w.base,
+                                       w.unit_first, w.unit_desc, w.work_counter, scan_gmax);
                 }
             }
         } else if (half)
             hipLaunchKernelGGL((bin_scatter_kernel<DIM, F, true>), SCATTER_GRID(plan), dim3(ScatterThreads<DIM, F, 1>::value),
                                stage_bytes(plan), s, lt, plan, cptr, w.gT, w.cursor, w.cnt, cps, cnt_rows,
                                reinterpret_cast<typename ItemSel<F, true>::type *>(w.items), s0, hi, NP, zacc, first_idx,
-                               w.unit_first, cstride);
+                               w.totals, cstride, w.base, w.unit_first, w.unit_desc, w.work_counter, scan_gmax);
         else if (use_fx)
             hipLaunchKernelGGL((bin_scatter_kernel<DIM, F, false>), SCATTER_GRID(plan), dim3(ScatterThreads<DIM, F, 0>::value),
                                stage_bytes(plan), s, lt, plan, cptr, w.gT, w.cursor, w.cnt, cps, cnt_rows,
-                               reinterpret_cast<Item<F> *>(w.items), s0, hi, NP, zacc, first_idx, w.unit_first, cstride);
+                               reinterpret_cast<Item<F> *>(w.items), s0, hi, NP, zacc, first_idx, w.totals, cstride, w.base, w.unit_first,
+                               w.unit_desc, w.work_counter, scan_gmax);
         else
             hipLaunchKernelGGL((bin_scatter_kernel<DIM, F, false, false>), SCATTER_GRID(plan), dim3(ScatterThreads<DIM, F, 0>::value),
                                stage_bytes(plan), s, lt, plan, cptr, w.gT, w.cursor, w.cnt, cps, cnt_rows,
-                               reinterpret_cast<Item<F> *>(w.items), s0, hi, NP, zacc, first_idx, w.unit_first, cstride);
+                               reinterpret_cast<Item<F> *>(w.items), s0, hi, NP, zacc, first_idx, w.totals, cstride, w.base, w.unit_first,
+                               w.unit_desc, w.work_counter, scan_gmax);
         SHACIRA_CHECK_LAUNCH();
-        if (fork) SHACIRA_CHECK(hipStreamWaitEvent(s, ss->join, 0));
-        if (brick_mode == 2) {
+        if (fork) {
+            SHACIRA_CHECK(hipStreamWaitEvent(s, ss->join, 0));
+            fork_guard.disarm();
+        }
+        if (brick_mode == 2 && (brick_split == 0 || brick_high.nlev > 0)) {
+            const BrickPlan &part = brick_split > 0 ? brick_high : brick;
+            if (!fork_signalled) SHACIRA_CHECK(hipEventRecord(bss->bfork, s));
+            SHACIRA_CHECK(hipStreamWaitEvent(bss->stream, bss->bfork, 0));
+            brick_guard.arm(s, bss->stream, bss->bjoin);
             if (fork_signalled) {
-                SHACIRA_CHECK(hipStreamWaitEvent(bss->stream, bss->bfork, 0));
-                SHACIRA_CHECK(launch_brick(bss->stream, bss->bjoin));
+                SHACIRA_CHECK(launch_brick(part, bss->stream, bss->bjoin));
             } else {
-                SHACIRA_CHECK(fork_brick());
+                SHACIRA_CHECK(launch_brick(part, bss->stream));
+                SHACIRA_CHECK(hipEventRecord(bss->bjoin, bss->stream));
             }
         }
         const uint64_t max_items = (uint64_t)(hi - s0) * plan.nbl * NPAIR +
@@ -794,8 +886,11 @@
                                reinterpret_cast<const Item<F> *>(w.items), acc, fa, headroom, wc);
         SHACIRA_CHECK_LAUNCH();
     }
-    if (brick_mode == 0) SHACIRA_CHECK(launch_brick(s));
-    if (brick_mode > 0) SHACIRA_CHECK(hipStreamWaitEvent(s, bss->bjoin, 0));
+    if (brick_mode == 0) SHACIRA_CHECK(launch_brick(brick, s));
+    if (brick_mode > 0) {
+        SHACIRA_CHECK(hipStreamWaitEvent(s, bss->bjoin, 0));
+        brick_guard.disarm();
+    }
     if (direct_half) {
         hipLaunchKernelGGL(f32_to_f16_skip_kernel, dim3(128, (uint32_t)L), dim3(256), 0, s, acc, half_table, first_idx, lt,
                            whole, w.unit_first, F);
diff --git a/shacira_amd/csrc/internal.h b/shacira_amd/csrc/internal.h
--- a/shacira_amd/csrc/internal.h
+++ b/shacira_amd/csrc/internal.h
@@ -192,6 +192,7 @@
     int bwd_brick_hi = -1;
     int bwd_brick_fork = 2;
     int bwd_brick_span = 0;
+    int bwd_brick_split = -1;
     int bwd_ext_fork = 1;
     int coord_variant = -1;
     int fwd_direct = -1;
```

Result: slower. 1.386 billion (-1.9%).
